# mhrice/RemFx

Hardware: AMD Instinct MI355X
Metric: audio-seconds/sec fwd+bwd (whole job) (higher is better)
Workload: dtype bf16 (fp32 accumulate); 1 GPU; Hybrid Demucs (cfg/model/demucs.yaml) train step, +exp=chorus_aug model=demucs; clips_per_gpu=64, global_batch=64, clip_samples=262144, parallelism=dp1, rccl_ranks=0, ranks=1, streams=4

## Files before the change

include/remfx_hip.h:

```cpp
#ifndef REMFX_HIP_H
#define REMFX_HIP_H

#include <stdint.h>

#ifdef __cplusplus
extern "C" {
#endif

#define RFX_ABI_VERSION 1

enum rfx_act {
  RFX_ACT_NONE = 0,
  RFX_ACT_RELU = 1,
  RFX_ACT_GELU = 2,
  RFX_ACT_TANH = 3,
  RFX_ACT_PRELU = 4,
  RFX_ACT_LEAKY = 5,
  RFX_ACT_SIGMOID = 6
};

typedef struct rfx_ktab_entry {
  int32_t off;
  int32_t da;
  int32_t db;
  int32_t flags;
} rfx_ktab_entry;

typedef struct rfx_gemm_desc {
  int32_t N, M, K;
  int32_t OA, OB;
  int32_t IA, IB;
  int32_t SA, SB;
  int32_t Mpad, Kpad;
  int32_t out_a0, out_b0, out_sa, out_sb;
  int32_t R;
  int32_t mg_log, mg_axis, mg_len, mg_off;
  int32_t Kpad_t, gpt, ntaps, gpt2;
  int64_t in_ns, in_as, in_bs;
  int64_t out_ns, out_cs, out_as, out_bs;
  int64_t in_cs, in_extent;
  int32_t in_bf16, out_bf16;
  int32_t halo_nt, halo_rows, halo_w, halo_da0, halo_db0, halo_pad;
} rfx_gemm_desc;

typedef struct rfx_epilogue {
  const float* bias;
  int32_t act;
  const float* act_param;
  const float* res;
  int64_t res_ns, res_cs, res_as, res_bs;
  int32_t act2;
  int32_t bwd;
  float* gparam;
  double* stat_sums;
  int32_t stat_slots;
  float* glu_out;
  int64_t glu_ns;
} rfx_epilogue;

enum rfx_gemm_prec { RFX_PREC_F32 = 0, RFX_PREC_BF16X3 = 1, RFX_PREC_BF16 = 2 };

int rfx_pack_a(const float* w, const int32_t* woff, int64_t w_ms, int32_t M, int32_t K,
               int32_t Mpad, int32_t Kpad, int32_t prec, float* apack, void* stream);
int rfx_unpack_add(const float* dapack, const int32_t* woff, int64_t w_ms, int32_t M, int32_t K,
                   int32_t Kpad, float* dw, int32_t splits, void* stream);
int rfx_unpack_add_bias(const float* dapack, const int32_t* woff, int64_t w_ms, int32_t M, int32_t K, int32_t Kpad, float* dw,
                        int32_t bias_col, float* db, int32_t splits, void* stream);
int rfx_unpack_set(const float* dapack, const int32_t* woff, int64_t w_ms, int32_t M, int32_t K,
                   int32_t Kpad, float* dw, int32_t splits, void* stream);
int rfx_unpack_col(const float* dapack, int32_t M, int32_t Kpad, int32_t col, int32_t splits, float* out, void* stream);

int rfx_gemm_fwd(const rfx_gemm_desc* d, const float* apack, const rfx_ktab_entry* ktab,
                 const float* in, float* out, const rfx_epilogue* epi,
                 const float* apack2, const rfx_ktab_entry* ktab2, int32_t K2, int32_t Kpad2,
                 const float* in2 ,
                 int32_t prec ,
                 void* stream);

int rfx_gemm_wgrad(const rfx_gemm_desc* d, const rfx_ktab_entry* ktab, const float* in,
                   const float* g, float* dapack, int64_t ws_floats, int32_t* splits_out, int32_t prec, void* stream);

enum rfx_stft_out {
  RFX_STFT_COMPLEX = 0,
  RFX_STFT_CAC = 1,
  RFX_STFT_MAG = 2,
  RFX_STFT_POW = 3,
  RFX_STFT_MAGPOW = 4,
  RFX_STFT_COMPLEX_FM = 5
};
typedef struct rfx_stft_desc {
  int32_t R, T;
  int32_t n_fft, hop, win;
  int32_t bins;
  int32_t frame0;
  int32_t frames_out;
  int32_t mode;
  int32_t extra_pad_l, extra_pad_r;
  int32_t in_mode;
  int32_t in_offset;
  int32_t herm;
  float scale;
  float eps, alpha;
  int32_t accum;
} rfx_stft_desc;

int rfx_fft_analysis(const rfx_stft_desc* d, const float* x, const float* window, const float* mul,
                     float* out, void* stream);
int64_t rfx_fft_synthesis_ws(const rfx_stft_desc* d);
int rfx_fft_synthesis(const rfx_stft_desc* d, const float* spec, const float* window, const float* mul,
                      float* ws, float* out, void* stream);

int rfx_lstm_pack_bytes(int32_t H);
int rfx_lstm_ws_bytes(int32_t H);
int rfx_lstm_pack(const float* whh, int32_t H, void* pack, void* stream);
int rfx_lstm_cat_params(const float* w_ih, const float* w_ih_r, const float* b_ih, const float* b_hh, const float* b_ih_r,
                        const float* b_hh_r, int32_t H, int32_t Cin, float* wcat, float* bcat, void* stream);
int rfx_lstm_grad_scatter(const float* dwcat, const float* dbcat, int32_t H, int32_t Cin, float* g_w_ih, float* g_w_ih_r,
                          float* g_b_ih, float* g_b_hh, float* g_b_ih_r, float* g_b_hh_r, void* stream);
int rfx_lstm_local(int32_t H, int32_t Bn, int32_t prec, int32_t bwd);
int rfx_lstm_pack_local(const float* whh, int32_t H, void* pack, void* stream);
int rfx_lstm_fwd(const float* xp, const void* pack, int32_t T, int32_t Bn, int32_t H, float* out, float* gates,
                 float* cstate, void* ws, int32_t prec, void* stream);
int rfx_lstm_bwd(const float* gout, const void* pack, const float* gates, const float* cstate, int32_t T,
                 int32_t Bn, int32_t H, float* dG, void* ws, int32_t prec, void* stream);
int rfx_lstm_set_local(int32_t fwd_max_sequences, int32_t bwd_max_sequences);

int rfx_act_fwd(const float* x, float* y, int64_t n, int32_t act, void* stream);
int rfx_act_bwd(const float* x, const float* gy, float* gx, int64_t n, int32_t act, void* stream);
int rfx_act_add_fwd(const float* x, const float* res, float* y, int64_t n, int32_t act, void* stream);
int rfx_act_rows(const float* x, int64_t xs0, int64_t xs1, int64_t xs2, const float* gy, int64_t gs0, int64_t gs1,
                 int64_t gs2, float* out, int64_t os0, int64_t os1, int64_t os2, int32_t D0, int32_t D1, int32_t D2,
                 int32_t T, int32_t act, void* stream);
int rfx_act_rows16(const void* x, int64_t xs0, int64_t xs1, int64_t xs2, const float* gy, int64_t gs0, int64_t gs1,
                   int64_t gs2, void* out, int64_t os0, int64_t os1, int64_t os2, int32_t D0, int32_t D1, int32_t D2,
                   int32_t T, int32_t act, void* stream);
int rfx_mul(const float* a, const float* b, float* y, int64_t n, void* stream);
int rfx_prelu_fwd(const float* x, const float* slope, float* y, int64_t N, int64_t C, int64_t L, void* stream);
int rfx_prelu_bwd(const float* x, const float* gy, const float* slope, float* gx, double* ws, float* gslope,
                  int64_t N, int64_t C, int64_t L, void* stream);

int64_t rfx_channel_sum_ws(const float* x, int32_t N, int32_t C, int32_t A, int32_t B, int64_t ns, int64_t cs, int64_t as, int64_t bs);
int rfx_channel_sum(const float* x, int32_t N, int32_t C, int32_t A, int32_t B, int64_t ns, int64_t cs,
                    int64_t as, int64_t bs, double* ws, float* out, void* stream);

int rfx_add_bcast(const float* x, const float* y, float* out, int64_t N, int32_t C, int32_t A, int32_t B,
                  int64_t yn, int64_t yc, int64_t ya, int64_t yb, float alpha, void* stream);
int rfx_row_moments_slots(int64_t L);
int rfx_row_moments(const float* x, int32_t R, int64_t L, double* sums, float* mean, float* stdv, float eps, float* coef_a,
                    float* coef_b, void* stream);
int rfx_row_affine(const float* x, const float* a, const float* b, float* out, int32_t R, int64_t L, void* stream);

int rfx_dropout(const float* x, float* out, int64_t n, float p, uint64_t seed, void* stream);

int rfx_span_mask(float* x, int32_t R, int32_t F, int32_t T, const int32_t* f0, const int32_t* f1, const int32_t* t0,
                  const int32_t* t1, void* stream);

int rfx_blstm_frames(const float* src, const float* skip, float* dst, int32_t B, int32_t C, int32_t T, int32_t nfr,
                     int32_t width, int32_t stride, int32_t mode, void* stream);

#define RFX_L1_SLOTS 512
int rfx_l1_sum(const float* a, const float* b, int64_t n, double* ws, float scale, float* out, void* stream);

int rfx_localstate_fwd(const float* q, const float* k, const float* cont, const float* qd, int32_t B, int32_t heads,
                       int32_t ch, int32_t T, int32_t nd, float* w, float* out, void* stream);
int rfx_localstate_bwd(const float* q, const float* k, const float* cont, const float* qd, const float* w,
                       const float* gout, int32_t B, int32_t heads, int32_t ch, int32_t T, int32_t nd, float* dq, float* dk,
                       float* dcont, float* dqd, void* stream);

int rfx_localstate_mfma_ok(int32_t B, int32_t heads, int32_t ch, int32_t T, int32_t nd);
int rfx_localstate_mfma_fwd(const float* q, const float* k, const float* cont, const float* qd, int32_t B, int32_t heads,
                            int32_t ch, int32_t T, int32_t nd, float* out, void* stream);
int rfx_localstate_mfma_bwd(const float* q, const float* k, const float* cont, const float* qd, const float* gout, int32_t B,
                            int32_t heads, int32_t ch, int32_t T, int32_t nd, float* dq, float* dk, float* dcont, float* dqd,
                            float* stat , void* stream);
int rfx_localstate_gen_fwd(const float* q, const float* k, const float* cont, const float* qd, int32_t B, int32_t heads,
                           int32_t ch, int32_t T, int32_t nd, float* stat, float* out, void* stream);
int rfx_localstate_gen_bwd(const float* q, const float* k, const float* cont, const float* qd, float* stat, const float* out,
                           const float* gout, int32_t B, int32_t heads, int32_t ch, int32_t T, int32_t nd, float* dq, float* dk,
                           float* dcont, float* dqd, void* stream);

int rfx_fx_distortion(const float* x, float* y, int32_t B, int64_t T, const float* gain , void* stream);
int rfx_fx_delay(const float* x, float* y, int32_t B, int64_t T, const int32_t* delay_samples, const float* feedback,
                 const float* mix, void* stream);
int rfx_fx_chorus(const float* x, float* y, int32_t B, int64_t T, float sample_rate, const float* rate_hz, const float* depth,
                  const float* centre_delay_ms, const float* feedback, const float* mix, void* stream);
int rfx_fx_compressor(const float* x, float* y, float* env_ws , int32_t B, int64_t T,
                      const float* threshold_lin, const float* ratio, const float* c_attack, const float* c_release, void* stream);
int rfx_fx_reverb(const float* x, float* y, int32_t B, int64_t T, int32_t sample_rate, const float* damp, const float* feedback,
                  const float* wet1, const float* dry, void* stream);
int rfx_fx_loudness(const float* x, int32_t B, int64_t T, int32_t chunk, int32_t hop_len, int32_t nhop, int32_t nblk,
                    double inv_block, const double* coef, float target_lufs, double* hop_ws, float* lufs, float* gain, void* stream);
int rfx_fx_scale(const float* x, float* y, int32_t B, int64_t T, const float* gain, void* stream);

int rfx_dconv_layer_ok(int32_t C, int32_t T, int32_t dil);
int rfx_dconv_layer_fwd(const float* x, float* out, int32_t N, int32_t C, int32_t T, int32_t dil, const float* w1, const float* b1,
                        const float* gn1w, const float* gn1b, const float* w2, const float* b2, const float* gn2w,
                        const float* gn2b, const float* scale, float eps, void* h16, void* z16, float* a_out, float* stats,
                        void* stream);
int rfx_dconv_layer_bwd_rows(int32_t N);
int rfx_dconv_layer_bwd(const float* x, const float* g, float* gx, int32_t N, int32_t C, int32_t T, int32_t dil, const float* w1,
                        const float* b1, const float* gn1w, const float* gn1b, const float* w2, const float* b2, const float* gn2w,
                        const float* gn2b, const float* scale, float eps, void* dz_bf16, float* a_out, void* dh_bf16, float* partial,
                        void* stream);

int rfx_gemm_fwd_variant(const rfx_gemm_desc* d, const rfx_epilogue* epi, int32_t two_phase, int32_t prec);

int rfx_mha_fwd(const float* q, const float* k, const float* v, int32_t B, int32_t heads, int32_t ch, int32_t T, float* stat,
                float* out, void* stream);
int rfx_mha_bwd(const float* q, const float* k, const float* v, float* stat, const float* out, const float* gout, int32_t B,
                int32_t heads, int32_t ch, int32_t T, float* dq, float* dk, float* dv, void* stream);

int rfx_groupnorm_fwd(const float* x, const float* gamma, const float* beta, int32_t N, int32_t C, int32_t S,
                      int32_t G, float eps, int32_t mode, const float* res, const float* scale,
                      double* sums ,
                      int32_t sums_given, float* mean, float* rstd, float* y, void* stream);
int rfx_groupnorm_stat_chunks(int32_t C, int32_t S, int32_t G);
int64_t rfx_norm_bwd_work_floats(int32_t N, int32_t C, int32_t S, int32_t G);
int rfx_groupnorm_bwd(const float* x, const float* gamma, const float* beta, const float* mean,
                      const float* rstd, const float* gy, int32_t N, int32_t C, int32_t S, int32_t G,
                      int32_t mode, const float* scale, float* work, float* dx, float* dgamma, float* dbeta,
                      float* dscale, void* stream);

int rfx_groupnorm_fwd_x16(const void* x, const float* gamma, const float* beta, int32_t N, int32_t C, int32_t S, int32_t G,
                          float eps, int32_t mode, const float* res, const float* scale, double* sums, int32_t sums_given,
                          float* mean, float* rstd, float* y, void* stream);
int rfx_groupnorm_bwd_x16(const void* x, const float* gamma, const float* beta, const float* mean, const float* rstd,
                          const float* gy, int32_t N, int32_t C, int32_t S, int32_t G, int32_t mode, const float* scale,
                          float* work, void* dx, float* dgamma, float* dbeta, float* dscale, void* stream);
int rfx_batchnorm_stat_slots(int32_t N, int32_t S);
int rfx_batchnorm_fwd(const float* x, const float* gamma, const float* beta, int32_t N, int32_t C, int32_t S,
                      float eps, int32_t mode, int32_t use_given_stats, double* sums, float* mean, float* rstd,
                      float* y, void* stream);
int rfx_batchnorm_bwd(const float* x, const float* gamma, const float* beta, const float* mean,
                      const float* rstd, const float* gy, int32_t N, int32_t C, int32_t S, int32_t mode,
                      float* work, float* dx, float* dgamma, float* dbeta, void* stream);
int rfx_avgpool2d_fwd(const float* x, float* y, int64_t NC, int32_t H, int32_t W, int32_t kh, int32_t kw,
                      void* stream);
int rfx_avgpool2d_bwd(const float* gy, float* gx, int64_t NC, int32_t H, int32_t W, int32_t kh, int32_t kw,
                      void* stream);
int rfx_glu_fwd(const float* x, float* y, int64_t N, int64_t C, int64_t S, void* stream);
int rfx_glu_bwd(const float* x, const float* gy, float* gx, int64_t N, int64_t C, int64_t S, void* stream);
int rfx_glu_bwd_bf16(const void* x, const float* gy, void* gx, int64_t N, int64_t C, int64_t S, void* stream);

int64_t rfx_cplx_slots(int32_t N, int64_t S);
int rfx_cplx_moments(const float* x, int32_t N, int32_t C, int64_t S, double* ws, double* sums, void* stream);
int rfx_cplx_coef_fwd(const double* sums, double inv_count, const float* stats_in, const float* Wrr, const float* Wri,
                      const float* Wii, const float* Br, const float* Bi, float eps, int32_t C, float* coef, float* stats_out,
                      float* RMr, float* RMi, float* RVrr, float* RVri, float* RVii, float momentum, void* stream);
int rfx_cplx_coef_bwd(const double* sums, double inv_count, const float* stats_in, const float* Wrr, const float* Wri,
                      const float* Wii, const float* Br, const float* Bi, float eps, int32_t C, const float* gcoef, float* gw,
                      float* cm, void* stream);
int rfx_cplx_moments_bwd(const float* x, const float* coef, int32_t N, int32_t C, int64_t S, float* gx, void* stream);
int rfx_cplx_affine_act_fwd(const float* x, const float* coef, int32_t N, int32_t C, int64_t S, float slope,
                            float* out, int64_t out_ns, int64_t out_im_off, void* stream);
int rfx_cplx_affine_act_bwd(const float* x, const float* coef, const float* gy, int64_t gy_ns, int64_t gy_im_off,
                            int32_t N, int32_t C, int64_t S, float slope, float* gx, double* ws, float* gcoef, void* stream);
int rfx_bound_mask_fwd(const float* m, const float* tf, float* out, int32_t N, int64_t P, int64_t m_ns,
                       int64_t tf_ns, int64_t out_ns, void* stream);
int rfx_bound_mask_bwd(const float* m, const float* tf, const float* gout, float* gm, int32_t N, int64_t P,
                       int64_t m_ns, int64_t tf_ns, int64_t g_ns, int64_t gm_ns, void* stream);

int rfx_phase_mask_fwd(const float* mag, const float* xc, float* out, int64_t n, void* stream);
int rfx_phase_mask_bwd(const float* xc, const float* gout, float* gmag, int64_t n, void* stream);

#define RFX_STFT_REDUCE_SLOTS 64
int rfx_stft_loss_reduce(const float* xc, const float* yc, int32_t R, int64_t n, float eps, double* ws, float* sums,
                         void* stream);
int rfx_stft_loss_grad(const float* xc, const float* yc, int32_t R, int64_t n, float eps,
                       const float* sums, float w_sc, float w_lm, const float* gup, float* gxc, void* stream);
int64_t rfx_stft_pair_loss_ws(const rfx_stft_desc* d);
int rfx_stft_pair_loss(const rfx_stft_desc* d, const float* x, const float* y, const float* window, float eps, double* ws, float* sums,
                       float* xspec, float* ymag, void* stream);
int rfx_stft_loss_grad_m(const float* xc, const float* ymag, int32_t R, int64_t n, float eps, const float* sums, float w_sc,
                         float w_lm, const float* gup, float* gxc, void* stream);
int rfx_fft_synthesis_lossgrad(const rfx_stft_desc* d, const float* xspec, const float* ymag, const float* sums, float w_sc,
                               float w_lm, float eps, const float* gup, const float* window, float* ws, float* out, void* stream);
int rfx_l1_grad(const float* a, const float* b, int64_t n, float w, const float* gup, float* g, void* stream);
#define RFX_SISDR_SLOTS 128
int rfx_sisdr_sums(const float* x, const float* t, int32_t R, int64_t L, int64_t x_rs, int64_t t_rs,
                   double* ws, double* sums, void* stream);
int rfx_sisdr_finish(const double* sums, int32_t R, int64_t L, int32_t zero_mean, double eps, float* out, void* stream);
int rfx_mrstft_combine(const float* const* sums, const int64_t* n, int32_t nres, int32_t R, int32_t per_example_sc, float* out,
                       void* stream);

int rfx_zero(void* p, int64_t nbytes, void* stream);
#define RFX_SUMSQ_SLOTS 4096
int rfx_sumsq(const float* g, int64_t n, double* ws, double* out, void* stream);
int rfx_clip_coef(const double* sumsq, float max_norm, float pre, float* coef, float* norm_out, void* stream);
int rfx_adamw_step(float* p, const float* g, float* m, float* v, int64_t n, float lr, float b1, float b2,
                   float eps, float wd, int32_t step, const float* gscale, void* stream);

typedef struct rfx_cl_tensor {
  void* p;
  int64_t ns, as;
  int32_t bs, c0;
} rfx_cl_tensor;

enum rfx_cl_epi {
  RFX_CL_STORE = 0,
  RFX_CL_GELU = 1,
  RFX_CL_GLU = 2,
  RFX_CL_DGELU = 3,
  RFX_CL_STORE_CM = 5,
  RFX_CL_DGLU = 4
};

typedef struct rfx_cl_conv_desc {
  rfx_cl_tensor in;
  int32_t N, IA, IB, OA, OB, SA;
  int32_t NTR, NCH, NTC, KS;
  int32_t da0, da_step;
  int32_t db0, db_step;
  int32_t wrapb;
  const void* apack;
  int32_t M, BM;
  int32_t mode;
  int32_t G, g_off, OAo, Co;
  const float* bias;
  const float* rowadd;
  rfx_cl_tensor out0, out1, aux0, res;
  void* cm_out;
  int64_t cm_ns, cm_cs, cm_as;
  int32_t cm_fold;
} rfx_cl_conv_desc;
int rfx_cl_conv(const rfx_cl_conv_desc* d, void* stream);
int rfx_cl_pack(const float* src, const int32_t* idx, int64_t n, void* dst, void* stream);
int rfx_cl_from_cm(const void* src, int32_t src_bf16, int64_t s_ns, int64_t s_cs, int64_t s_as, int32_t N, int32_t C, int32_t A,
                   int32_t B, const rfx_cl_tensor* dst, const rfx_cl_tensor* res, const rfx_cl_tensor* aux, int32_t mode, void* stream);
int rfx_cl_to_cm(const rfx_cl_tensor* src, int32_t N, int32_t C, int32_t A, int32_t B, void* dst, int32_t dst_bf16, int64_t d_ns,
                 int64_t d_cs, int64_t d_as, const void* aux16, void* stream);
int rfx_cl_im2col_s4(const float* src, int64_t s_ns, int64_t s_cs, int64_t s_as, int32_t N, int32_t Cs, int32_t IA, int32_t IB, int32_t OA,
                     int32_t OB, int32_t along_b, void* dst, void* stream);
int rfx_cl_im2col_fm(const float* src, const float* coef_a, const float* coef_b, int32_t N, int32_t F, int32_t bins, void* dst, void* stream);
int rfx_fm_cm_affine(const float* in, float* out, const float* coef_a, const float* coef_b, int32_t N, int32_t bins, int32_t F, int32_t to_fm,
                     void* stream);
int rfx_cl_dgelu(const void* g, const void* z, void* out, int64_t n, void* stream);
int rfx_cl_dglu(const void* g, const void* zab, void* out, int64_t npos, int32_t C, void* stream);

typedef struct rfx_cl_wgrad_desc {
  rfx_cl_tensor p, q;
  int32_t N, OA, IA, B;
  int32_t SA, da0, NTR;
  int32_t NTC, db0, db_step;
  int32_t M, Cq, CW;
  int32_t RW, WK;
  int32_t S, ahead, bias;
  int32_t PW;
  float* ws;
} rfx_cl_wgrad_desc;
int64_t rfx_cl_wgrad_ws_floats(const rfx_cl_wgrad_desc* d);
int rfx_cl_wgrad(const rfx_cl_wgrad_desc* d, void* stream);
int rfx_cl_wgrad_reduce(const float* ws, const int32_t* map, int64_t nmap, int32_t S, int32_t DT, int32_t RW, int32_t WK, float* dw,
                        int64_t wn, float* db, int32_t accumulate, void* stream);

typedef struct rfx_cl_dconv_desc {
  const void* x;
  const void* gy;
  void* y;
  void* a; void* hpre; float* stats;
  void* dz; void* dh; float* partial;
  const void* w1p; const void* w2p; const void* w2dp; const void* w1dp;
  const float *b1, *g1w, *g1b, *b2, *g2w, *g2b, *scale;
  int32_t S, C, H, dil, grid, x_or_gy_ok;
  float eps;
  int32_t TPS;
  float* tsum; float* sums;
  float* pg_dst[5];
} rfx_cl_dconv_desc;
int rfx_cl_dconv_ok(int32_t C, int32_t H, int32_t T, int32_t backward);
int rfx_cl_dconv_fwd(const rfx_cl_dconv_desc* d, void* stream);
int rfx_cl_dconv_bwd(const rfx_cl_dconv_desc* d, float* pgrad, void* stream);

int rfx_cl_rowsum(const rfx_cl_tensor* x, int32_t N, int32_t A, int32_t B, int32_t C, int32_t G, float scale, float* partial, float* out,
                  int32_t accumulate, void* stream);

int rfx_abi_version(void);
int rfx_gemm_pick_r(int32_t M, int32_t K);

#ifdef __cplusplus
}
#endif
#endif
```

remfx_amd/_lib.py:

```python
import ctypes as C
import glob
import os
import subprocess

_HERE = os.path.dirname(os.path.abspath(__file__))
_ROOT = os.path.dirname(_HERE)
CSRC = os.path.join(_HERE, "csrc")
INCLUDE = os.path.join(_ROOT, "include")
LIBDIR = os.path.join(_HERE, "_C")
LIBPATH = os.environ.get("RFX_LIBPATH_DEV") or os.path.join(LIBDIR, "libremfx_hip.so")

HIPCC_FLAGS = ["--offload-arch=gfx950", "-O3", "-std=c++17", "-fPIC", "-ffp-contract=fast",
               "-I" + INCLUDE, "-I" + CSRC]


def sources():
    return sorted(glob.glob(os.path.join(CSRC, "*.hip")))


def _stale():
    if not os.path.exists(LIBPATH):
        return True
    t = os.path.getmtime(LIBPATH)
    deps = sources() + glob.glob(os.path.join(CSRC, "*.h")) + glob.glob(os.path.join(INCLUDE, "*.h"))
    return any(os.path.getmtime(p) > t for p in deps)


def build(force=False, verbose=False):
    if not force and not _stale():
        return LIBPATH
    hipcc = os.environ.get("HIPCC", "/opt/rocm/bin/hipcc")
    os.makedirs(LIBDIR, exist_ok=True)
    objs = []
    hdr_t = max([os.path.getmtime(p) for p in glob.glob(os.path.join(CSRC, "*.h")) +
                 glob.glob(os.path.join(INCLUDE, "*.h"))] or [0])
    procs = []
    for src in sources():
        obj = os.path.join(LIBDIR, os.path.basename(src)[:-4] + ".o")
        objs.append(obj)
        if (not force and os.path.exists(obj) and os.path.getmtime(obj) > os.path.getmtime(src)
                and os.path.getmtime(obj) > hdr_t):
            continue
        cmd = [hipcc] + HIPCC_FLAGS + ["-c", src, "-o", obj]
        if verbose:
            print(" ".join(cmd))
        procs.append((src, subprocess.Popen(cmd, stdout=subprocess.PIPE, stderr=subprocess.STDOUT)))
    for src, p in procs:
        out, _ = p.communicate()
        if p.returncode != 0:
            raise RuntimeError(f"hipcc failed on {src}:\n{out.decode()}")
    cmd = [hipcc, "--offload-arch=gfx950", "-shared", "-fPIC", "-o", LIBPATH] + objs
    r = subprocess.run(cmd, stdout=subprocess.PIPE, stderr=subprocess.STDOUT)
    if r.returncode != 0:
        raise RuntimeError(f"link failed:\n{r.stdout.decode()}")
    return LIBPATH


class KtabEntry(C.Structure):
    _fields_ = [("off", C.c_int32), ("da", C.c_int32), ("db", C.c_int32), ("flags", C.c_int32)]


class GemmDesc(C.Structure):
    _fields_ = [(n, C.c_int32) for n in ("N", "M", "K", "OA", "OB", "IA", "IB", "SA", "SB", "Mpad",
                                         "Kpad", "out_a0", "out_b0", "out_sa", "out_sb", "R", "mg_log", "mg_axis", "mg_len", "mg_off",
                                         "Kpad_t", "gpt", "ntaps", "gpt2")] + \
               [(n, C.c_int64) for n in ("in_ns", "in_as", "in_bs", "out_ns", "out_cs", "out_as", "out_bs", "in_cs", "in_extent")] + \
               [("in_bf16", C.c_int32), ("out_bf16", C.c_int32)] + \
               [(n, C.c_int32) for n in ("halo_nt", "halo_rows", "halo_w", "halo_da0", "halo_db0", "halo_pad")]


class Epilogue(C.Structure):
    _fields_ = [("bias", C.c_void_p), ("act", C.c_int32), ("act_param", C.c_void_p),
                ("res", C.c_void_p), ("res_ns", C.c_int64), ("res_cs", C.c_int64),
                ("res_as", C.c_int64), ("res_bs", C.c_int64), ("act2", C.c_int32), ("bwd", C.c_int32),
                ("gparam", C.c_void_p), ("stat_sums", C.c_void_p), ("stat_slots", C.c_int32),
                ("glu_out", C.c_void_p), ("glu_ns", C.c_int64)]


class StftDesc(C.Structure):
    _fields_ = [(n, C.c_int32) for n in ("R", "T", "n_fft", "hop", "win", "bins", "frame0", "frames_out",
                                         "mode", "extra_pad_l", "extra_pad_r", "in_mode", "in_offset",
                                         "herm")] + \
               [(n, C.c_float) for n in ("scale", "eps", "alpha")] + [("accum", C.c_int32)]


class ClTensor(C.Structure):
    _fields_ = [("p", C.c_void_p), ("ns", C.c_int64), ("as_", C.c_int64), ("bs", C.c_int32), ("c0", C.c_int32)]


class ClConvDesc(C.Structure):
    _fields_ = [("inp", ClTensor)] + \
               [(n, C.c_int32) for n in ("N", "IA", "IB", "OA", "OB", "SA", "NTR", "NCH", "NTC", "KS", "da0", "da_step", "db0",
                                         "db_step", "wrapb")] + \
               [("apack", C.c_void_p)] + \
               [(n, C.c_int32) for n in ("M", "BM", "mode", "G", "g_off", "OAo", "Co")] + \
               [("bias", C.c_void_p), ("rowadd", C.c_void_p), ("out0", ClTensor), ("out1", ClTensor), ("aux0", ClTensor), ("res", ClTensor),
                ("cm_out", C.c_void_p), ("cm_ns", C.c_int64), ("cm_cs", C.c_int64), ("cm_as", C.c_int64), ("cm_fold", C.c_int32)]


class ClDconvDesc(C.Structure):
    _fields_ = [(n, C.c_void_p) for n in ("x", "gy", "y", "a", "hpre", "stats", "dz", "dh", "partial", "w1p", "w2p", "w2dp", "w1dp",
                                          "b1", "g1w", "g1b", "b2", "g2w", "g2b", "scale")] + \
               [(n, C.c_int32) for n in ("S", "C", "H", "dil", "grid", "x_or_gy_ok")] + [("eps", C.c_float), ("TPS", C.c_int32), ("tsum", C.c_void_p), ("sums", C.c_void_p), ("pg_dst", C.c_void_p * 5)]


class ClWgradDesc(C.Structure):
    _fields_ = [("p", ClTensor), ("q", ClTensor)] + \
               [(n, C.c_int32) for n in ("N", "OA", "IA", "B", "SA", "da0", "NTR", "NTC", "db0", "db_step", "M", "Cq", "CW", "RW", "WK",
                                         "S", "ahead", "bias", "PW")] + \
               [("ws", C.c_void_p)]


_P, _I32, _I64 = C.c_void_p, C.c_int32, C.c_int64
SIGNATURES = {
    "rfx_abi_version": [],
    "rfx_gemm_pick_r": [_I32, _I32],
    "rfx_pack_a": [_P, _P, _I64, _I32, _I32, _I32, _I32, _I32, _P, _P],
    "rfx_unpack_add": [_P, _P, _I64, _I32, _I32, _I32, _P, _I32, _P],
    "rfx_unpack_add_bias": [_P, _P, _I64, _I32, _I32, _I32, _P, _I32, _P, _I32, _P],
    "rfx_unpack_set": [_P, _P, _I64, _I32, _I32, _I32, _P, _I32, _P],
    "rfx_unpack_col": [_P, _I32, _I32, _I32, _I32, _P, _P],
    "rfx_gemm_fwd": [C.POINTER(GemmDesc), _P, _P, _P, _P, C.POINTER(Epilogue), _P, _P, _I32, _I32, _P, _I32, _P],
    "rfx_gemm_fwd_variant": [C.POINTER(GemmDesc), C.POINTER(Epilogue), _I32, _I32],
    "rfx_gemm_wgrad": [C.POINTER(GemmDesc), _P, _P, _P, _P, _I64, C.POINTER(C.c_int32), _I32, _P],
    "rfx_fft_analysis": [C.POINTER(StftDesc), _P, _P, _P, _P, _P],
    "rfx_fft_synthesis_ws": [C.POINTER(StftDesc)],
    "rfx_fft_synthesis": [C.POINTER(StftDesc), _P, _P, _P, _P, _P, _P],
    "rfx_stft_loss_reduce": [_P, _P, _I32, _I64, C.c_float, _P, _P, _P],
    "rfx_stft_loss_grad": [_P, _P, _I32, _I64, C.c_float, _P, C.c_float, C.c_float, _P, _P, _P],
    "rfx_stft_loss_grad_m": [_P, _P, _I32, _I64, C.c_float, _P, C.c_float, C.c_float, _P, _P, _P],
    "rfx_stft_pair_loss_ws": [C.POINTER(StftDesc)],
    "rfx_stft_pair_loss": [C.POINTER(StftDesc), _P, _P, _P, C.c_float, _P, _P, _P, _P, _P],
    "rfx_fft_synthesis_lossgrad": [C.POINTER(StftDesc), _P, _P, _P, C.c_float, C.c_float, C.c_float, _P, _P, _P, _P, _P],
    "rfx_l1_grad": [_P, _P, _I64, C.c_float, _P, _P, _P],
    "rfx_sisdr_sums": [_P, _P, _I32, _I64, _I64, _I64, _P, _P, _P],
    "rfx_sisdr_finish": [_P, _I32, _I64, _I32, C.c_double, _P, _P],
    "rfx_mrstft_combine": [_P, _P, _I32, _I32, _I32, _P, _P],
    "rfx_zero": [_P, _I64, _P],
    "rfx_sumsq": [_P, _I64, _P, _P, _P],
    "rfx_clip_coef": [_P, C.c_float, C.c_float, _P, _P, _P],
    "rfx_adamw_step": [_P, _P, _P, _P, _I64, C.c_float, C.c_float, C.c_float, C.c_float, C.c_float, _I32, _P, _P],
    "rfx_groupnorm_stat_chunks": [_I32, _I32, _I32],
    "rfx_norm_bwd_work_floats": [_I32, _I32, _I32, _I32],
    "rfx_batchnorm_stat_slots": [_I32, _I32],
    "rfx_groupnorm_fwd": [_P, _P, _P, _I32, _I32, _I32, _I32, C.c_float, _I32, _P, _P, _P, _I32, _P, _P, _P, _P],
    "rfx_groupnorm_bwd": [_P, _P, _P, _P, _P, _P, _I32, _I32, _I32, _I32, _I32, _P, _P, _P, _P, _P, _P, _P],
    "rfx_groupnorm_fwd_x16": [_P, _P, _P, _I32, _I32, _I32, _I32, C.c_float, _I32, _P, _P, _P, _I32, _P, _P, _P, _P],
    "rfx_groupnorm_bwd_x16": [_P, _P, _P, _P, _P, _P, _I32, _I32, _I32, _I32, _I32, _P, _P, _P, _P, _P, _P, _P],
    "rfx_batchnorm_fwd": [_P, _P, _P, _I32, _I32, _I32, C.c_float, _I32, _I32, _P, _P, _P, _P, _P],
    "rfx_batchnorm_bwd": [_P, _P, _P, _P, _P, _P, _I32, _I32, _I32, _I32, _P, _P, _P, _P, _P],
    "rfx_avgpool2d_fwd": [_P, _P, _I64, _I32, _I32, _I32, _I32, _P],
    "rfx_avgpool2d_bwd": [_P, _P, _I64, _I32, _I32, _I32, _I32, _P],
    "rfx_cplx_slots": [_I32, _I64],
    "rfx_cplx_moments": [_P, _I32, _I32, _I64, _P, _P, _P],
    "rfx_cplx_moments_bwd": [_P, _P, _I32, _I32, _I64, _P, _P],
    "rfx_cplx_coef_fwd": [_P, C.c_double, _P, _P, _P, _P, _P, _P, C.c_float, _I32, _P, _P, _P, _P, _P, _P, _P, C.c_float, _P],
    "rfx_cplx_coef_bwd": [_P, C.c_double, _P, _P, _P, _P, _P, _P, C.c_float, _I32, _P, _P, _P, _P],
    "rfx_cplx_affine_act_fwd": [_P, _P, _I32, _I32, _I64, C.c_float, _P, _I64, _I64, _P],
    "rfx_cplx_affine_act_bwd": [_P, _P, _P, _I64, _I64, _I32, _I32, _I64, C.c_float, _P, _P, _P, _P],
    "rfx_bound_mask_fwd": [_P, _P, _P, _I32, _I64, _I64, _I64, _I64, _P],
    "rfx_bound_mask_bwd": [_P, _P, _P, _P, _I32, _I64, _I64, _I64, _I64, _I64, _P],
    "rfx_phase_mask_fwd": [_P, _P, _P, _I64, _P],
    "rfx_phase_mask_bwd": [_P, _P, _P, _I64, _P],
    "rfx_glu_fwd": [_P, _P, _I64, _I64, _I64, _P],
    "rfx_glu_bwd": [_P, _P, _P, _I64, _I64, _I64, _P],
    "rfx_glu_bwd_bf16": [_P, _P, _P, _I64, _I64, _I64, _P],
    "rfx_act_fwd": [_P, _P, _I64, _I32, _P],
    "rfx_act_bwd": [_P, _P, _P, _I64, _I32, _P],
    "rfx_act_add_fwd": [_P, _P, _P, _I64, _I32, _P],
    "rfx_act_rows": [_P, _I64, _I64, _I64, _P, _I64, _I64, _I64, _P, _I64, _I64, _I64, _I32, _I32, _I32, _I32, _I32, _P],
    "rfx_act_rows16": [_P, _I64, _I64, _I64, _P, _I64, _I64, _I64, _P, _I64, _I64, _I64, _I32, _I32, _I32, _I32, _I32, _P],
    "rfx_mul": [_P, _P, _P, _I64, _P],
    "rfx_prelu_fwd": [_P, _P, _P, _I64, _I64, _I64, _P],
    "rfx_prelu_bwd": [_P, _P, _P, _P, _P, _P, _I64, _I64, _I64, _P],
    "rfx_l1_sum": [_P, _P, _I64, _P, C.c_float, _P, _P],
    "rfx_add_bcast": [_P, _P, _P, _I64, _I32, _I32, _I32, _I64, _I64, _I64, _I64, C.c_float, _P],
    "rfx_localstate_fwd": [_P, _P, _P, _P, _I32, _I32, _I32, _I32, _I32, _P, _P, _P],
    "rfx_localstate_bwd": [_P, _P, _P, _P, _P, _P, _I32, _I32, _I32, _I32, _I32, _P, _P, _P, _P, _P],
    "rfx_dconv_layer_ok": [_I32, _I32, _I32],
    "rfx_dconv_layer_bwd_rows": [_I32],
    "rfx_dconv_layer_bwd": [_P, _P, _P, _I32, _I32, _I32, _I32, _P, _P, _P, _P, _P, _P, _P, _P, _P, C.c_float, _P, _P, _P, _P, _P],
    "rfx_dconv_layer_fwd": [_P, _P, _I32, _I32, _I32, _I32, _P, _P, _P, _P, _P, _P, _P, _P, _P, C.c_float, _P, _P, _P, _P, _P],
    "rfx_fx_distortion": [_P, _P, _I32, _I64, _P, _P],
    "rfx_fx_delay": [_P, _P, _I32, _I64, _P, _P, _P, _P],
    "rfx_fx_chorus": [_P, _P, _I32, _I64, C.c_float, _P, _P, _P, _P, _P, _P],
    "rfx_fx_compressor": [_P, _P, _P, _I32, _I64, _P, _P, _P, _P, _P],
    "rfx_fx_reverb": [_P, _P, _I32, _I64, _I32, _P, _P, _P, _P, _P],
    "rfx_fx_loudness": [_P, _I32, _I64, _I32, _I32, _I32, _I32, C.c_double, _P, C.c_float, _P, _P, _P, _P],
    "rfx_fx_scale": [_P, _P, _I32, _I64, _P, _P],
    "rfx_localstate_gen_fwd": [_P, _P, _P, _P, _I32, _I32, _I32, _I32, _I32, _P, _P, _P],
    "rfx_localstate_gen_bwd": [_P, _P, _P, _P, _P, _P, _P, _I32, _I32, _I32, _I32, _I32, _P, _P, _P, _P, _P],
    "rfx_mha_fwd": [_P, _P, _P, _I32, _I32, _I32, _I32, _P, _P, _P],
    "rfx_mha_bwd": [_P, _P, _P, _P, _P, _P, _I32, _I32, _I32, _I32, _P, _P, _P, _P],
    "rfx_localstate_mfma_ok": [_I32, _I32, _I32, _I32, _I32],
    "rfx_localstate_mfma_fwd": [_P, _P, _P, _P, _I32, _I32, _I32, _I32, _I32, _P, _P],
    "rfx_localstate_mfma_bwd": [_P, _P, _P, _P, _P, _I32, _I32, _I32, _I32, _I32, _P, _P, _P, _P, _P, _P],
    "rfx_blstm_frames": [_P, _P, _P, _I32, _I32, _I32, _I32, _I32, _I32, _I32, _P],
    "rfx_span_mask": [_P, _I32, _I32, _I32, _P, _P, _P, _P, _P],
    "rfx_dropout": [_P, _P, _I64, C.c_float, C.c_uint64, _P],
    "rfx_row_moments_slots": [_I64],
    "rfx_row_moments": [_P, _I32, _I64, _P, _P, _P, C.c_float, _P, _P, _P],
    "rfx_row_affine": [_P, _P, _P, _P, _I32, _I64, _P],
    "rfx_lstm_pack_bytes": [_I32],
    "rfx_lstm_pack": [_P, _I32, _P, _P],
    "rfx_lstm_cat_params": [_P, _P, _P, _P, _P, _P, _I32, _I32, _P, _P, _P],
    "rfx_lstm_grad_scatter": [_P, _P, _I32, _I32, _P, _P, _P, _P, _P, _P, _P],
    "rfx_lstm_local": [_I32, _I32, _I32, _I32],
    "rfx_lstm_pack_local": [_P, _I32, _P, _P],
    "rfx_lstm_ws_bytes": [_I32],
    "rfx_lstm_fwd": [_P, _P, _I32, _I32, _I32, _P, _P, _P, _P, _I32, _P],
    "rfx_lstm_bwd": [_P, _P, _P, _P, _I32, _I32, _I32, _P, _P, _I32, _P],
    "rfx_lstm_set_local": [_I32, _I32],
    "rfx_channel_sum_ws": [_P, _I32, _I32, _I32, _I32, _I64, _I64, _I64, _I64],
    "rfx_channel_sum": [_P, _I32, _I32, _I32, _I32, _I64, _I64, _I64, _I64, _P, _P, _P],
    "rfx_cl_conv": [C.POINTER(ClConvDesc), _P],
    "rfx_cl_pack": [_P, _P, _I64, _P, _P],
    "rfx_cl_wgrad_ws_floats": [_P],
    "rfx_cl_wgrad": [_P, _P],
    "rfx_cl_wgrad_reduce": [_P, _P, _I64, _I32, _I32, _I32, _I32, _P, _I64, _P, _I32, _P],
    "rfx_cl_from_cm": [_P, _I32, _I64, _I64, _I64, _I32, _I32, _I32, _I32, C.POINTER(ClTensor), C.POINTER(ClTensor), C.POINTER(ClTensor),
                       _I32, _P],
    "rfx_cl_rowsum": [C.POINTER(ClTensor), _I32, _I32, _I32, _I32, _I32, C.c_float, _P, _P, _I32, _P],
    "rfx_cl_to_cm": [C.POINTER(ClTensor), _I32, _I32, _I32, _I32, _P, _I32, _I64, _I64, _I64, _P, _P],
    "rfx_cl_dgelu": [_P, _P, _P, _I64, _P],
    "rfx_cl_dglu": [_P, _P, _P, _I64, _I32, _P],
    "rfx_cl_im2col_s4": [_P, _I64, _I64, _I64, _I32, _I32, _I32, _I32, _I32, _I32, _I32, _P, _P],
    "rfx_cl_im2col_fm": [_P, _P, _P, _I32, _I32, _I32, _P, _P],
    "rfx_fm_cm_affine": [_P, _P, _P, _P, _I32, _I32, _I32, _I32, _P],
    "rfx_cl_dconv_ok": [_I32, _I32, _I32, _I32],
    "rfx_cl_dconv_fwd": [_P, _P],
    "rfx_cl_dconv_bwd": [_P, _P, _P],
}

_RET64 = {"rfx_cl_wgrad_ws_floats", "rfx_cplx_slots", "rfx_norm_bwd_work_floats", "rfx_stft_pair_loss_ws", "rfx_channel_sum_ws", "rfx_fft_synthesis_ws"}
_lib = None


def lib():
    global _lib
    if _lib is not None:
        return _lib
    import torch
    if not os.path.exists(LIBPATH):
        raise RuntimeError(
            f"{LIBPATH} not found: run `python -c 'import __graft_entry__ as g; g.build()'` "
            "(hipcc --offload-arch=gfx950).  remfx_amd has no CPU fallback.")
    L = C.CDLL(LIBPATH)
    for name, argtypes in SIGNATURES.items():
        fn = getattr(L, name)
        fn.argtypes = argtypes
        fn.restype = C.c_int64 if name in _RET64 else C.c_int
    if L.rfx_abi_version() != 1:
        raise RuntimeError("libremfx_hip ABI version mismatch")
    _lib = L
    return L


def check(rc, what):
    if rc != 0:
        raise RuntimeError(f"{what} failed with code {rc}")
```

remfx_amd/csrc/lstm.hip:

```cpp
#include "common.h"
#include <stdlib.h>

typedef __bf16 bf16x8 __attribute__((ext_vector_type(8)));

__device__ __forceinline__ uint32_t lstm_bf16_rne(float f) {
  const uint32_t u = __float_as_uint(f);
  return (u + 0x7fffu + ((u >> 16) & 1u)) >> 16;
}
__device__ __forceinline__ float lstm_sigmoid(float x) { return __builtin_amdgcn_rcpf(1.f + __expf(-x)); }
__device__ __forceinline__ float lstm_tanh(float x) { return 2.f * __builtin_amdgcn_rcpf(1.f + __expf(-2.f * x)) - 1.f; }
__device__ __forceinline__ void split_hi_lo(float v, unsigned short& hi, unsigned short& lo) {
  const uint32_t u = __float_as_uint(v);
  const float r = v - __uint_as_float(u & 0xffff0000u);
  hi = (unsigned short)(u >> 16);
  lo = (unsigned short)((__float_as_uint(r) + 0x8000u) >> 16);
}

__global__ void lstm_pack_kernel(const float* __restrict__ whh, int H, uint4* __restrict__ fwdA, uint4* __restrict__ bwdA) {
  const int nub = H / 32, nks = H / 16, nks4 = 4 * H / 16;
  const int64_t nf = (int64_t)nub * 4 * nks * 64, nb = (int64_t)nub * nks4 * 64;
  for (int64_t idx = (int64_t)blockIdx.x * blockDim.x + threadIdx.x; idx < nf + nb; idx += (int64_t)gridDim.x * blockDim.x) {
    uint32_t hi[4] = {0, 0, 0, 0}, lo[4] = {0, 0, 0, 0};
    const bool f = idx < nf;
    const int64_t i = f ? idx : idx - nf;
    const int lane = (int)(i & 63);
    int64_t r = i >> 6;
#pragma unroll
    for (int q = 0; q < 8; ++q) {
      float v;
      if (f) {
        const int ks = (int)(r % nks), tl = (int)((r / nks) % 2), ub = (int)(r / (2 * nks)), m = lane & 31;
        v = whh[(int64_t)((2 * tl + (m >> 4)) * H + 16 * ub + (m & 15)) * H + 16 * ks + 8 * (lane >> 5) + q];
      } else {
        const int ks = (int)(r % nks4), ub = (int)(r / nks4);
        v = whh[(int64_t)(16 * ks + 8 * (lane >> 5) + q) * H + 32 * ub + (lane & 31)];
      }
      const uint32_t h = lstm_bf16_rne(v);
      const uint32_t l = lstm_bf16_rne(v - __uint_as_float(h << 16));
      hi[q >> 1] |= h << (16 * (q & 1));
      lo[q >> 1] |= l << (16 * (q & 1));
    }
    uint4* dst = f ? fwdA : bwdA;
    const int64_t n = f ? nf : nb;
    dst[i] = make_uint4(hi[0], hi[1], hi[2], hi[3]);
    dst[n + i] = make_uint4(lo[0], lo[1], lo[2], lo[3]);
  }
}


#define RFX_LSTM_MAX_WAVES 768
#define RFX_LSTM_SPIN_LIMIT (1 << 22)

struct LstmArgs {
  const float* xp;
  const uint4* packA;
  float* out;
  float* gates;
  float* cstate;
  const float* gout;
  float* dG;
  uint64_t* xch;
  uint32_t* ctr;
  int32_t* err;
  int64_t pack_stride;
  int T, Bn, H, P;
  int tile0, nclusters;
};

__device__ __forceinline__ bool lstm_wait(const uint32_t* ctr, uint32_t target) {
  for (int it = 0; it < RFX_LSTM_SPIN_LIMIT; ++it) {
    const uint32_t v = __hip_atomic_load(ctr, __ATOMIC_RELAXED, __HIP_MEMORY_SCOPE_AGENT);
    if (__builtin_amdgcn_readfirstlane(v) >= target) return true;
    __builtin_amdgcn_s_sleep(1);
  }
  return false;
}
__device__ __forceinline__ void lstm_arrive(uint32_t* ctr, int lane) {
  __builtin_amdgcn_s_waitcnt(0x0F70);
  if (lane == 0) __hip_atomic_fetch_add(ctr, 1u, __ATOMIC_RELAXED, __HIP_MEMORY_SCOPE_AGENT);
}
__device__ __forceinline__ bf16x8 lstm_xch_load(const uint64_t* p) {
  const uint64_t a = __hip_atomic_load(p, __ATOMIC_RELAXED, __HIP_MEMORY_SCOPE_AGENT);
  const uint64_t b = __hip_atomic_load(p + 1, __ATOMIC_RELAXED, __HIP_MEMORY_SCOPE_AGENT);
  const uint4 v = make_uint4((uint32_t)a, (uint32_t)(a >> 32), (uint32_t)b, (uint32_t)(b >> 32));
  return __builtin_bit_cast(bf16x8, v);
}
__device__ __forceinline__ void lstm_xch_store(uint64_t* phi, uint64_t* plo, float v0, float v1, float v2, float v3) {
  unsigned short h0, h1, h2, h3, l0, l1, l2, l3;
  split_hi_lo(v0, h0, l0); split_hi_lo(v1, h1, l1); split_hi_lo(v2, h2, l2); split_hi_lo(v3, h3, l3);
  const uint64_t hi = (uint64_t)h0 | ((uint64_t)h1 << 16) | ((uint64_t)h2 << 32) | ((uint64_t)h3 << 48);
  const uint64_t lo = (uint64_t)l0 | ((uint64_t)l1 << 16) | ((uint64_t)l2 << 32) | ((uint64_t)l3 << 48);
  __hip_atomic_store(phi, hi, __ATOMIC_RELAXED, __HIP_MEMORY_SCOPE_AGENT);
  __hip_atomic_store(plo, lo, __ATOMIC_RELAXED, __HIP_MEMORY_SCOPE_AGENT);
}

__device__ __forceinline__ bool lstm_ids(const LstmArgs& a, int nwc, int& cluster, int& ub) {
  const int w = blockIdx.x, j = w >> 3;
  cluster = (j / nwc) * 8 + (w & 7);
  ub = j % nwc;
  return cluster < a.nclusters;
}

typedef uint32_t lstm_u32x4 __attribute__((ext_vector_type(4)));
typedef const __attribute__((address_space(1))) lstm_u32x4* lstm_gptr_t;

struct LstmAFrag { uint4 h[2], l[2]; };

extern __shared__ __attribute__((aligned(16))) unsigned char lstm_smem[];

__device__ __forceinline__ void lstm_fetch_lds(const uint64_t* src, int n, int lane) {
  for (int i = 0; i < n; ++i)
    __builtin_amdgcn_global_load_lds((const __attribute__((address_space(1))) void*)(src + (i * 64 + lane) * 2),
                                     (__attribute__((address_space(3))) void*)(lstm_smem + i * 1024), 16, 0,
                                     16 );
}

__device__ __forceinline__ void lstm_fetch_lds_hi(const uint64_t* src, int nks, int lane) {
  for (int ks = 0; ks < nks; ++ks)
    __builtin_amdgcn_global_load_lds((const __attribute__((address_space(1))) void*)(src + (2 * ks * 64 + lane) * 2),
                                     (__attribute__((address_space(3))) void*)(lstm_smem + ks * 2048), 16, 0,
                                     16 );
}
__device__ __forceinline__ void lstm_xch_store_hi(uint64_t* phi, float v0, float v1, float v2, float v3) {
  const uint64_t hi = (uint64_t)rfx_cvt_pk_bf16(v0, v1) | ((uint64_t)rfx_cvt_pk_bf16(v2, v3) << 32);
  __hip_atomic_store(phi, hi, __ATOMIC_RELAXED, __HIP_MEMORY_SCOPE_AGENT);
}

template <int D, int NKS, bool LO>
__global__ __launch_bounds__(64) __attribute__((amdgpu_waves_per_eu(1, 1))) void lstm_fwd_kernel(const LstmArgs a) {
  int cluster, ub;
  if (!lstm_ids(a, a.H / 16, cluster, ub)) return;
  const int H = a.H, Bn = a.Bn, T = a.T, P = a.P;
  const int dir = cluster & 1, row0 = (a.tile0 + (cluster >> 1)) * 32;
  const int lane = threadIdx.x, l31 = lane & 31, hh = lane >> 5;
  const int nks = NKS ? NKS : H / 16, nwc = nks;
  const int row = row0 + l31;
  const bool rvalid = row < Bn;
  const int rowc = rvalid ? row : 0;
  const float* __restrict__ xp = a.xp + (int64_t)dir * 4 * H * P;
  const int nf = nwc * 2 * nks * 64;
  uint64_t abase = (uint64_t)(a.packA + (int64_t)dir * a.pack_stride + ub * 2 * nks * 64);
  lstm_gptr_t Ahi = (lstm_gptr_t)abase;
  lstm_gptr_t Alo = Ahi + nf;
  float* outp = a.out + (int64_t)dir * H * P;
  float* gsave = a.gates ? a.gates + (int64_t)dir * 4 * H * P : nullptr;
  float* csave = a.gates ? a.cstate + (int64_t)dir * H * P : nullptr;
  const int bufw = nks * 256;
  uint64_t* xch = a.xch + (int64_t)cluster * 2 * bufw;
  uint32_t* ctr = a.ctr + cluster * 16;
  const uint32_t uP = (uint32_t)P, HP = (uint32_t)H * uP;
  const uint32_t ubase = (uint32_t)(16 * ub + 4 * hh) * uP + (uint32_t)rowc;
  const uint32_t lane16 = (uint32_t)lane * 16u;
  auto loadA = [&](LstmAFrag& f, int ks) {
#pragma unroll
    for (int tl = 0; tl < 2; ++tl) {
      f.h[tl] = __builtin_bit_cast(uint4, *(lstm_gptr_t)((uint64_t)(Ahi + (tl * nks + ks) * 64) + lane16));
      if (LO) f.l[tl] = __builtin_bit_cast(uint4, *(lstm_gptr_t)((uint64_t)(Alo + (tl * nks + ks) * 64) + lane16));
    }
  };
  auto loadB = [&](bf16x8& bh, bf16x8& bl, int ks) {
    bh = *reinterpret_cast<const bf16x8*>(lstm_smem + ks * 2048 + lane * 16);
    if (LO) bl = *reinterpret_cast<const bf16x8*>(lstm_smem + ks * 2048 + 1024 + lane * 16);
  };
  auto mma = [&](f32x16* acc, const LstmAFrag& f, const bf16x8 bh, const bf16x8 bl) {
#pragma unroll
    for (int tl = 0; tl < 2; ++tl)
      acc[tl] = __builtin_amdgcn_mfma_f32_32x32x16_bf16(__builtin_bit_cast(bf16x8, f.h[tl]), bh, acc[tl], 0, 0, 0);
    if (LO) {
#pragma unroll
      for (int tl = 0; tl < 2; ++tl)
        acc[tl] = __builtin_amdgcn_mfma_f32_32x32x16_bf16(__builtin_bit_cast(bf16x8, f.h[tl]), bl, acc[tl], 0, 0, 0);
#pragma unroll
      for (int tl = 0; tl < 2; ++tl)
        acc[tl] = __builtin_amdgcn_mfma_f32_32x32x16_bf16(__builtin_bit_cast(bf16x8, f.l[tl]), bh, acc[tl], 0, 0, 0);
    }
  };
  float c[8];
#pragma unroll
  for (int r = 0; r < 8; ++r) c[r] = 0.f;
  f32x16 acc[2];
  LstmAFrag f[D];
#pragma unroll
  for (int d = 0; d < D; ++d) loadA(f[d], d);
  float xpv[4][8];
  {
    const uint32_t o0 = ubase + (uint32_t)((dir == 0 ? 0 : T - 1) * Bn);
#pragma unroll
    for (int g = 0; g < 4; ++g)
#pragma unroll
      for (int r = 0; r < 8; ++r) xpv[g][r] = xp[o0 + (uint32_t)g * HP + (uint32_t)((r & 3) + 8 * (r >> 2)) * uP];
  }
  for (int s = 0; s < T; ++s) {
    if (NKS) { asm volatile("" : "+s"(abase)); Ahi = (lstm_gptr_t)abase; Alo = Ahi + nf; }

    const int t = dir == 0 ? s : T - 1 - s;
    const uint32_t o0 = ubase + (uint32_t)(t * Bn);
#pragma unroll
    for (int tl = 0; tl < 2; ++tl)
#pragma unroll
      for (int r = 0; r < 16; ++r) acc[tl][r] = 0.f;
    if (s > 0) {
      if (!lstm_wait(ctr, (uint32_t)(nwc * s))) { *a.err = 1; return; }
      if (LO) lstm_fetch_lds(xch + ((s - 1) & 1) * bufw, 2 * nks, lane);
      else lstm_fetch_lds_hi(xch + ((s - 1) & 1) * bufw, nks, lane);
      __builtin_amdgcn_s_waitcnt(0x0F70);
    }
    if (s > 0) {
      bf16x8 bh[2], bl[2];
      loadB(bh[0], bl[0], 0);
      auto kstep = [&](int ks) {
#pragma unroll
        for (int d = 0; d < D; ++d) {
          const int k1 = ks + d + 1 == nks ? 0 : ks + d + 1;
          loadB(bh[(d + 1) & 1], bl[(d + 1) & 1], k1);
          mma(acc, f[d], bh[d & 1], bl[d & 1]);
          if (!(NKS && D == NKS)) {
            const int kn = ks + d + D;
            loadA(f[d], kn >= nks ? kn - nks : kn);
          }
          __builtin_amdgcn_sched_barrier(0);
        }
      };
      if (NKS) {
#pragma unroll
        for (int ks = 0; ks < NKS; ks += D) kstep(ks);
      } else {
        for (int ks = 0; ks < nks; ks += D) kstep(ks);
      }
    }
    uint64_t* hw = xch + (s & 1) * bufw;
    float hv[8], gi[8], gf[8], gc[8], go[8];
#pragma unroll
    for (int r = 0; r < 8; ++r) {
      const float ig = lstm_sigmoid(acc[0][r] + xpv[0][r]), fg = lstm_sigmoid(acc[0][r + 8] + xpv[1][r]);
      const float gg = lstm_tanh(acc[1][r] + xpv[2][r]), og = lstm_sigmoid(acc[1][r + 8] + xpv[3][r]);
      c[r] = fg * c[r] + ig * gg;
      hv[r] = og * lstm_tanh(c[r]);
      gi[r] = ig; gf[r] = fg; gc[r] = gg; go[r] = og;
    }
    if (s + 1 < T) {
#pragma unroll
      for (int hb2 = 0; hb2 < 2; ++hb2) {
        const int r0 = 4 * hb2;
        uint64_t* d = hw + ((ub * 2) * 64 + l31 + 32 * hb2) * 2 + hh;
        if (LO) lstm_xch_store(d, d + 128, hv[r0], hv[r0 + 1], hv[r0 + 2], hv[r0 + 3]);
        else lstm_xch_store_hi(d, hv[r0], hv[r0 + 1], hv[r0 + 2], hv[r0 + 3]);
      }
      lstm_arrive(ctr, lane);
    }
    if (rvalid) {
#pragma unroll
      for (int r = 0; r < 8; ++r) {
        const uint32_t o = o0 + (uint32_t)((r & 3) + 8 * (r >> 2)) * uP;
        outp[o] = hv[r];
        if (gsave) {
          gsave[o] = gi[r]; gsave[o + HP] = gf[r]; gsave[o + 2 * HP] = gc[r]; gsave[o + 3 * HP] = go[r];
          csave[o] = c[r];
        }
      }
    }
    if (s + 1 < T) {
      const uint32_t on = ubase + (uint32_t)((dir == 0 ? s + 1 : T - 2 - s) * Bn);
#pragma unroll
      for (int g = 0; g < 4; ++g)
#pragma unroll
        for (int r = 0; r < 8; ++r) xpv[g][r] = xp[on + (uint32_t)g * HP + (uint32_t)((r & 3) + 8 * (r >> 2)) * uP];
    }
  }
}

template <int TPC, int NWC, bool LO, bool RES>
__global__ __launch_bounds__(64) __attribute__((amdgpu_waves_per_eu(1, 1))) void lstm_bwd_kernel(const LstmArgs a) {
  static_assert(!RES || NWC > 0, "resident weights need the compile-time tile count");
  int cluster, ub;
  if (!lstm_ids(a, a.H / 16, cluster, ub)) return;
  const int H = a.H, Bn = a.Bn, T = a.T, P = a.P;
  const int dir = cluster & 1, row0 = (a.tile0 + (cluster >> 1)) * 32;
  const int lane = threadIdx.x, l31 = lane & 31, hh = lane >> 5;
  const int nwc = NWC ? NWC : H / 32, nwv = 2 * nwc, nks = nwv, nks4 = 4 * nks;
  const int row = row0 + l31;
  const bool rvalid = row < Bn;
  const int rowc = rvalid ? row : 0;
  const int nf = nwc * 4 * nks * 64, nb = nwc * nks4 * 64;
  uint64_t abase = (uint64_t)(a.packA + (int64_t)dir * a.pack_stride + 2 * nf + ub * 64);
  lstm_gptr_t Ahi = (lstm_gptr_t)abase;
  lstm_gptr_t Alo = Ahi + nb;
  const float* __restrict__ gates = a.gates + (int64_t)dir * 4 * H * P;
  const float* __restrict__ cst = a.cstate + (int64_t)dir * H * P;
  float* __restrict__ dG = a.dG + (int64_t)dir * 4 * H * P;
  const float* __restrict__ goutp = a.gout + (int64_t)dir * H * P;
  const int bufw = nwv * nwv * 256;
  uint64_t* xch = a.xch + (int64_t)cluster * 2 * bufw;
  uint32_t* ctr = a.ctr + cluster * 16;
  const uint32_t uP = (uint32_t)P, HP = (uint32_t)H * uP;
  const uint32_t ubase = (uint32_t)(16 * ub + 4 * hh) * uP + (uint32_t)rowc;
  constexpr int RING = RES ? 4 * NWC : 4 * TPC;
  const int F = 4 * nwc;
  auto frag_index = [&](int fi) { const int ot = fi >> 2, g = fi & 3; return (ot * nks4 + g * nks) * 64 + lane; };
  uint4 wh[RING], wl[LO ? RING : 1];
#pragma unroll
  for (int i = 0; i < RING; ++i) {
    wh[i] = __builtin_bit_cast(uint4, Ahi[frag_index(i)]);
    if (LO) wl[i] = __builtin_bit_cast(uint4, Alo[frag_index(i)]);
  }
  float dcc[8], ct[8];
  float sg[4][8], cp[8], gy[8];
  {
    const uint32_t o0 = ubase + (uint32_t)((dir == 0 ? T - 1 : 0) * Bn);
    const uint32_t op0 = ubase + (uint32_t)((T > 1 ? (dir == 0 ? T - 2 : 1) : (dir == 0 ? T - 1 : 0)) * Bn);
#pragma unroll
    for (int r = 0; r < 8; ++r) {
      const uint32_t du = (uint32_t)((r & 3) + 8 * (r >> 2)) * uP;
      dcc[r] = 0.f;
      ct[r] = cst[o0 + du];
      sg[0][r] = gates[o0 + du]; sg[1][r] = gates[o0 + du + HP]; sg[2][r] = gates[o0 + du + 2 * HP]; sg[3][r] = gates[o0 + du + 3 * HP];
      cp[r] = cst[op0 + du];
      gy[r] = goutp[o0 + du];
    }
  }
  for (int s = T - 1; s >= 0; --s) {
    if (NWC && !RES) { asm volatile("" : "+s"(abase)); Ahi = (lstm_gptr_t)abase; Alo = Ahi + nb; }
    const int step = T - 1 - s;
    const int t = dir == 0 ? s : T - 1 - s;
    const uint32_t o0 = ubase + (uint32_t)(t * Bn);
    if (step > 0) {
      if (!lstm_wait(ctr, (uint32_t)(nwv * step))) { *a.err = 1; return; }
      lstm_fetch_lds(xch + ((step - 1) & 1) * bufw + ub * nwv * 256, 2 * nwv, lane);
      __builtin_amdgcn_s_waitcnt(0x0F70);
    }
    if (step > 0) {
      for (int p = 0; p < nwv; ++p)
#pragma unroll
        for (int jj = 0; jj < 2; ++jj) {
          const f32x4 v = *reinterpret_cast<const f32x4*>(lstm_smem + (p * 2 + jj) * 1024 + lane * 16);
          gy[4 * jj] += v[0]; gy[4 * jj + 1] += v[1]; gy[4 * jj + 2] += v[2]; gy[4 * jj + 3] += v[3];
        }
    }
#pragma unroll
    for (int r = 0; r < 8; ++r) {
      const float ig = sg[0][r], fg = sg[1][r], gg = sg[2][r], og = sg[3][r];
      const float cprev = s > 0 ? cp[r] : 0.f;
      const float th = lstm_tanh(ct[r]);
      const float dc = gy[r] * og * (1.f - th * th) + dcc[r];
      sg[3][r] = gy[r] * th * og * (1.f - og);
      sg[0][r] = dc * gg * ig * (1.f - ig);
      sg[1][r] = dc * cprev * fg * (1.f - fg);
      sg[2][r] = dc * ig * (1.f - gg * gg);
      dcc[r] = dc * fg;
      ct[r] = cp[r];
    }
    if (s > 0) {
      uint4 bh[4], bl[LO ? 4 : 1];
#pragma unroll
      for (int g = 0; g < 4; ++g) {
        uint32_t x0h[2], x0l[2], x1h[2], x1l[2];
#pragma unroll
        for (int e = 0; e < 2; ++e) {
          if (LO) {
            unsigned short h0, l0, h1, l1;
            split_hi_lo(sg[g][2 * e], h0, l0); split_hi_lo(sg[g][2 * e + 1], h1, l1);
            x0h[e] = (uint32_t)h0 | ((uint32_t)h1 << 16); x0l[e] = (uint32_t)l0 | ((uint32_t)l1 << 16);
            split_hi_lo(sg[g][4 + 2 * e], h0, l0); split_hi_lo(sg[g][4 + 2 * e + 1], h1, l1);
            x1h[e] = (uint32_t)h0 | ((uint32_t)h1 << 16); x1l[e] = (uint32_t)l0 | ((uint32_t)l1 << 16);
          } else {
            x0h[e] = rfx_cvt_pk_bf16(sg[g][2 * e], sg[g][2 * e + 1]);
            x1h[e] = rfx_cvt_pk_bf16(sg[g][4 + 2 * e], sg[g][4 + 2 * e + 1]);
            x0l[e] = x1l[e] = 0;
          }
        }
        uint32_t rh[2], rl[2] = {0, 0};
#pragma unroll
        for (int e = 0; e < 2; ++e) {
          rh[e] = (uint32_t)__shfl_xor((int)(hh ? x0h[e] : x1h[e]), 32, 64);
          if (LO) rl[e] = (uint32_t)__shfl_xor((int)(hh ? x0l[e] : x1l[e]), 32, 64);
        }
        bh[g] = hh ? make_uint4(rh[0], rh[1], x1h[0], x1h[1]) : make_uint4(x0h[0], x0h[1], rh[0], rh[1]);
        if (LO) bl[g] = hh ? make_uint4(rl[0], rl[1], x1l[0], x1l[1]) : make_uint4(x0l[0], x0l[1], rl[0], rl[1]);
      }
      uint64_t* gw = xch + (step & 1) * bufw;
      auto round = [&](int f0) {
        f32x16 acc[TPC];
#pragma unroll
        for (int tp = 0; tp < TPC; ++tp)
#pragma unroll
          for (int r = 0; r < 16; ++r) acc[tp][r] = 0.f;
#pragma unroll
        for (int g = 0; g < 4; ++g) {
          const bf16x8 Bh = __builtin_bit_cast(bf16x8, bh[g]), Bl = __builtin_bit_cast(bf16x8, bl[LO ? g : 0]);
#pragma unroll
          for (int tp = 0; tp < TPC; ++tp)
            acc[tp] = __builtin_amdgcn_mfma_f32_32x32x16_bf16(__builtin_bit_cast(bf16x8, wh[(RES ? f0 : 0) + tp * 4 + g]), Bh, acc[tp], 0, 0, 0);
          if (LO) {
#pragma unroll
            for (int tp = 0; tp < TPC; ++tp)
              acc[tp] = __builtin_amdgcn_mfma_f32_32x32x16_bf16(__builtin_bit_cast(bf16x8, wh[(RES ? f0 : 0) + tp * 4 + g]), Bl, acc[tp], 0, 0, 0);
#pragma unroll
            for (int tp = 0; tp < TPC; ++tp)
              acc[tp] = __builtin_amdgcn_mfma_f32_32x32x16_bf16(__builtin_bit_cast(bf16x8, wl[LO ? (RES ? f0 : 0) + tp * 4 + g : 0]), Bh, acc[tp], 0, 0, 0);
          }
          if (!RES) {
#pragma unroll
            for (int tp = 0; tp < TPC; ++tp) {
              const int i = tp * 4 + g;
              int fn = f0 + i + RING;
              fn = fn >= F ? fn - F : fn;
              wh[i] = __builtin_bit_cast(uint4, Ahi[frag_index(fn)]);
              if (LO) wl[LO ? i : 0] = __builtin_bit_cast(uint4, Alo[frag_index(fn)]);
            }
            __builtin_amdgcn_sched_barrier(0);
          }
        }
#pragma unroll
        for (int tp = 0; tp < TPC; ++tp) {
          const int ot = (f0 >> 2) + tp;
#pragma unroll
          for (int j = 0; j < 4; ++j) {
            uint64_t* d = gw + (int64_t)(((2 * ot + (j >> 1)) * nwv + ub) * 2 + (j & 1)) * 128 + lane * 2;
            const uint64_t v0 = (uint64_t)__float_as_uint(acc[tp][4 * j]) | ((uint64_t)__float_as_uint(acc[tp][4 * j + 1]) << 32);
            const uint64_t v1 = (uint64_t)__float_as_uint(acc[tp][4 * j + 2]) | ((uint64_t)__float_as_uint(acc[tp][4 * j + 3]) << 32);
            __hip_atomic_store(d, v0, __ATOMIC_RELAXED, __HIP_MEMORY_SCOPE_AGENT);
            __hip_atomic_store(d + 1, v1, __ATOMIC_RELAXED, __HIP_MEMORY_SCOPE_AGENT);
          }
        }
      };
      if (NWC) {
#pragma unroll
        for (int f0 = 0; f0 < 4 * NWC; f0 += 4 * TPC) round(f0);
      } else {
        for (int f0 = 0; f0 < F; f0 += 4 * TPC) round(f0);
      }
      lstm_arrive(ctr, lane);
    }
    if (rvalid) {
#pragma unroll
      for (int r = 0; r < 8; ++r) {
        const uint32_t o = o0 + (uint32_t)((r & 3) + 8 * (r >> 2)) * uP;
        dG[o] = sg[0][r]; dG[o + HP] = sg[1][r]; dG[o + 2 * HP] = sg[2][r]; dG[o + 3 * HP] = sg[3][r];
      }
    }
    if (s > 0) {
      const int s1 = s - 1, s2 = s1 > 0 ? s1 - 1 : 0;
      const uint32_t on = ubase + (uint32_t)((dir == 0 ? s1 : T - 1 - s1) * Bn);
      const uint32_t opn = ubase + (uint32_t)((dir == 0 ? s2 : T - 1 - s2) * Bn);
#pragma unroll
      for (int r = 0; r < 8; ++r) {
        const uint32_t du = (uint32_t)((r & 3) + 8 * (r >> 2)) * uP;
        sg[0][r] = gates[on + du]; sg[1][r] = gates[on + du + HP]; sg[2][r] = gates[on + du + 2 * HP]; sg[3][r] = gates[on + du + 3 * HP];
        cp[r] = cst[opn + du];
        gy[r] = goutp[on + du];
      }
    }
  }
}

typedef float lstm_f32x4 __attribute__((ext_vector_type(4)));

__global__ void lstm_pack_local_kernel(const float* __restrict__ whh, int H, uint4* __restrict__ dst) {
  const int nw = H / 16, nk = H / 32, nk4 = 4 * nk;
  const int64_t nf = (int64_t)nw * 4 * nk * 64, nb = (int64_t)nw * nk4 * 64;
  for (int64_t idx = (int64_t)blockIdx.x * blockDim.x + threadIdx.x; idx < nf + nb; idx += (int64_t)gridDim.x * blockDim.x) {
    const bool f = idx < nf;
    const int64_t i = f ? idx : idx - nf;
    const int lane = (int)(i & 63), row = lane & 15, kb = lane >> 4;
    int64_t r = i >> 6;
    uint32_t pk[4] = {0, 0, 0, 0};
#pragma unroll
    for (int j = 0; j < 8; ++j) {
      float v;
      if (f) {
        const int ks = (int)(r % nk), g = (int)((r / nk) % 4), w = (int)(r / (4 * nk));
        v = whh[(int64_t)(g * H + 16 * w + row) * H + 32 * ks + 8 * kb + j];
      } else {
        const int ks = (int)(r % nk4), w = (int)(r / nk4);
        v = whh[(int64_t)(32 * ks + 8 * kb + j) * H + 16 * w + row];
      }
      pk[j >> 1] |= lstm_bf16_rne(v) << (16 * (j & 1));
    }
    dst[idx] = make_uint4(pk[0], pk[1], pk[2], pk[3]);
  }
}
static int64_t lstm_local_uint4_per_dir(int H) { return (H <= 192) ? (int64_t)2 * (H / 16) * 4 * (H / 32) * 64 : 0; }

__device__ __forceinline__ void lstm_local_publish(unsigned char* buf, int k0, int sq, float v0, float v1, float v2, float v3) {
  const int ks = k0 >> 5, kk = k0 & 31;
  *reinterpret_cast<uint2*>(buf + ks * 1024 + (16 * (kk >> 3) + sq) * 16 + 2 * (kk & 7)) =
      make_uint2(rfx_cvt_pk_bf16(v0, v1), rfx_cvt_pk_bf16(v2, v3));
}
__device__ __forceinline__ void lstm_lds_barrier() { asm volatile("s_waitcnt lgkmcnt(0)\n\ts_barrier" ::: "memory"); }

template <int NW>
__global__ __launch_bounds__(64 * NW) __attribute__((amdgpu_waves_per_eu(3, 3))) void lstm_fwd_local_kernel(const LstmArgs a, const uint4* __restrict__ lpack,
                                                                                                             int64_t lstride) {
  constexpr int H = 16 * NW, NK = H / 32;
  const int cluster = blockIdx.x, dir = cluster & 1, tile = cluster >> 1;
  const int tid = threadIdx.x, w = __builtin_amdgcn_readfirstlane(tid >> 6), lane = tid & 63, sq = lane & 15, qb = lane >> 4;
  const int Bn = a.Bn, T = a.T, P = a.P;
  const int b = tile * 16 + sq;
  const bool rvalid = b < Bn;
  const int bc = rvalid ? b : 0;
  const float* __restrict__ xp = a.xp + (int64_t)dir * 4 * H * P;
  float* outp = a.out + (int64_t)dir * H * P;
  float* gsave = a.gates ? a.gates + (int64_t)dir * 4 * H * P : nullptr;
  float* csave = a.gates ? a.cstate + (int64_t)dir * H * P : nullptr;
  const uint32_t uP = (uint32_t)P, HP = (uint32_t)H * uP;
  const int u0 = 16 * w + 4 * qb;
  const uint32_t ubase = (uint32_t)u0 * uP + (uint32_t)bc;
  uint4 wf[4][NK];
  {
    const uint4* A = lpack + (int64_t)dir * lstride + (int64_t)w * 4 * NK * 64 + lane;
#pragma unroll
    for (int g = 0; g < 4; ++g)
#pragma unroll
      for (int ks = 0; ks < NK; ++ks) wf[g][ks] = A[(g * NK + ks) * 64];
  }
  float c[4] = {0.f, 0.f, 0.f, 0.f};
  float xpv[4][4];
  {
    const uint32_t o0 = ubase + (uint32_t)((dir == 0 ? 0 : T - 1) * Bn);
#pragma unroll
    for (int g = 0; g < 4; ++g)
#pragma unroll
      for (int r = 0; r < 4; ++r) xpv[g][r] = xp[o0 + (uint32_t)g * HP + (uint32_t)r * uP];
  }
  for (int s = 0; s < T; ++s) {
    const int t = dir == 0 ? s : T - 1 - s;
    const uint32_t o0 = ubase + (uint32_t)(t * Bn);
    lstm_f32x4 acc[4];
#pragma unroll
    for (int g = 0; g < 4; ++g) acc[g] = lstm_f32x4{0.f, 0.f, 0.f, 0.f};
    if (s > 0) {
      const unsigned char* hb = lstm_smem + ((s - 1) & 1) * (NK * 1024) + lane * 16;
#pragma unroll
      for (int ks = 0; ks < NK; ++ks) {
        const bf16x8 bh = *reinterpret_cast<const bf16x8*>(hb + ks * 1024);
#pragma unroll
        for (int g = 0; g < 4; ++g)
          acc[g] = __builtin_amdgcn_mfma_f32_16x16x32_bf16(__builtin_bit_cast(bf16x8, wf[g][ks]), bh, acc[g], 0, 0, 0);
      }
    }
    float hv[4], gi[4], gf[4], gc[4], go[4];
#pragma unroll
    for (int r = 0; r < 4; ++r) {
      const float ig = lstm_sigmoid(acc[0][r] + xpv[0][r]), fg = lstm_sigmoid(acc[1][r] + xpv[1][r]);
      const float gg = lstm_tanh(acc[2][r] + xpv[2][r]), og = lstm_sigmoid(acc[3][r] + xpv[3][r]);
      c[r] = fg * c[r] + ig * gg;
      hv[r] = og * lstm_tanh(c[r]);
      gi[r] = ig; gf[r] = fg; gc[r] = gg; go[r] = og;
    }
    if (s + 1 < T) {
      lstm_local_publish(lstm_smem + (s & 1) * (NK * 1024), u0, sq, hv[0], hv[1], hv[2], hv[3]);
      const uint32_t on = ubase + (uint32_t)((dir == 0 ? s + 1 : T - 2 - s) * Bn);
#pragma unroll
      for (int g = 0; g < 4; ++g)
#pragma unroll
        for (int r = 0; r < 4; ++r) xpv[g][r] = xp[on + (uint32_t)g * HP + (uint32_t)r * uP];
      lstm_lds_barrier();
    }
    if (rvalid) {
#pragma unroll
      for (int r = 0; r < 4; ++r) {
        const uint32_t o = o0 + (uint32_t)r * uP;
        outp[o] = hv[r];
        if (gsave) {
          gsave[o] = gi[r]; gsave[o + HP] = gf[r]; gsave[o + 2 * HP] = gc[r]; gsave[o + 3 * HP] = go[r];
          csave[o] = c[r];
        }
      }
    }
  }
}

template <int NW>
__global__ __launch_bounds__(64 * NW) __attribute__((amdgpu_waves_per_eu(3, 3))) void lstm_bwd_local_kernel(const LstmArgs a, const uint4* __restrict__ lpack,
                                                                                                             int64_t lstride) {
  constexpr int H = 16 * NW, NK = H / 32, NK4 = 4 * NK;
  const int cluster = blockIdx.x, dir = cluster & 1, tile = cluster >> 1;
  const int tid = threadIdx.x, w = __builtin_amdgcn_readfirstlane(tid >> 6), lane = tid & 63, sq = lane & 15, qb = lane >> 4;
  const int Bn = a.Bn, T = a.T, P = a.P;
  const int b = tile * 16 + sq;
  const bool rvalid = b < Bn;
  const int bc = rvalid ? b : 0;
  const float* __restrict__ gates = a.gates + (int64_t)dir * 4 * H * P;
  const float* __restrict__ cst = a.cstate + (int64_t)dir * H * P;
  float* __restrict__ dG = a.dG + (int64_t)dir * 4 * H * P;
  const float* __restrict__ goutp = a.gout + (int64_t)dir * H * P;
  const uint32_t uP = (uint32_t)P, HP = (uint32_t)H * uP;
  const int u0 = 16 * w + 4 * qb;
  const uint32_t ubase = (uint32_t)u0 * uP + (uint32_t)bc;
  uint4 wb[NK4];
  {
    const uint4* A = lpack + (int64_t)dir * lstride + (int64_t)NW * 4 * NK * 64 + (int64_t)w * NK4 * 64 + lane;
#pragma unroll
    for (int ks = 0; ks < NK4; ++ks) wb[ks] = A[ks * 64];
  }
  float dcc[4] = {0.f, 0.f, 0.f, 0.f}, ct[4], sg[4][4], cp[4], gy[4];
  {
    const uint32_t o0 = ubase + (uint32_t)((dir == 0 ? T - 1 : 0) * Bn);
    const uint32_t op0 = ubase + (uint32_t)((T > 1 ? (dir == 0 ? T - 2 : 1) : (dir == 0 ? T - 1 : 0)) * Bn);
#pragma unroll
    for (int r = 0; r < 4; ++r) {
      const uint32_t du = (uint32_t)r * uP;
      ct[r] = cst[o0 + du];
      sg[0][r] = gates[o0 + du]; sg[1][r] = gates[o0 + du + HP]; sg[2][r] = gates[o0 + du + 2 * HP]; sg[3][r] = gates[o0 + du + 3 * HP];
      cp[r] = cst[op0 + du];
      gy[r] = goutp[o0 + du];
    }
  }
  lstm_f32x4 rec = lstm_f32x4{0.f, 0.f, 0.f, 0.f};
  for (int s = T - 1; s >= 0; --s) {
    const int step = T - 1 - s;
    const int t = dir == 0 ? s : T - 1 - s;
    const uint32_t o0 = ubase + (uint32_t)(t * Bn);
#pragma unroll
    for (int r = 0; r < 4; ++r) {
      const float dh = gy[r] + rec[r];
      const float ig = sg[0][r], fg = sg[1][r], gg = sg[2][r], og = sg[3][r];
      const float cprev = s > 0 ? cp[r] : 0.f;
      const float th = lstm_tanh(ct[r]);
      const float dc = dh * og * (1.f - th * th) + dcc[r];
      sg[3][r] = dh * th * og * (1.f - og);
      sg[0][r] = dc * gg * ig * (1.f - ig);
      sg[1][r] = dc * cprev * fg * (1.f - fg);
      sg[2][r] = dc * ig * (1.f - gg * gg);
      dcc[r] = dc * fg;
      ct[r] = cp[r];
    }
    unsigned char* gb = lstm_smem + (step & 1) * (NK4 * 1024);
    if (s > 0) {
#pragma unroll
      for (int g = 0; g < 4; ++g) lstm_local_publish(gb, g * H + u0, sq, sg[g][0], sg[g][1], sg[g][2], sg[g][3]);
    }
    if (rvalid) {
#pragma unroll
      for (int r = 0; r < 4; ++r) {
        const uint32_t o = o0 + (uint32_t)r * uP;
        dG[o] = sg[0][r]; dG[o + HP] = sg[1][r]; dG[o + 2 * HP] = sg[2][r]; dG[o + 3 * HP] = sg[3][r];
      }
    }
    if (s > 0) {
      lstm_lds_barrier();
      lstm_f32x4 p[4];
#pragma unroll
      for (int q = 0; q < 4; ++q) p[q] = lstm_f32x4{0.f, 0.f, 0.f, 0.f};
#pragma unroll
      for (int ks = 0; ks < NK4; ++ks) {
        const bf16x8 bh = *reinterpret_cast<const bf16x8*>(gb + ks * 1024 + lane * 16);
        p[ks & 3] = __builtin_amdgcn_mfma_f32_16x16x32_bf16(__builtin_bit_cast(bf16x8, wb[ks]), bh, p[ks & 3], 0, 0, 0);
      }
      const int s1 = s - 1, s2 = s1 > 0 ? s1 - 1 : 0;
      const uint32_t on = ubase + (uint32_t)((dir == 0 ? s1 : T - 1 - s1) * Bn);
      const uint32_t opn = ubase + (uint32_t)((dir == 0 ? s2 : T - 1 - s2) * Bn);
#pragma unroll
      for (int r = 0; r < 4; ++r) {
        const uint32_t du = (uint32_t)r * uP;
        sg[0][r] = gates[on + du]; sg[1][r] = gates[on + du + HP]; sg[2][r] = gates[on + du + 2 * HP]; sg[3][r] = gates[on + du + 3 * HP];
        cp[r] = cst[opn + du];
        gy[r] = goutp[on + du];
      }
      rec = (p[0] + p[1]) + (p[2] + p[3]);
    }
  }
}

static int64_t lstm_cluster_uint4_per_dir(int H) {
  const int64_t nf = (int64_t)(H / 32) * 4 * (H / 16) * 64, nb = (int64_t)(H / 32) * (4 * H / 16) * 64;
  return 2 * nf + 2 * nb;
}
static int64_t lstm_pack_uint4_per_dir(int H) { return lstm_cluster_uint4_per_dir(H) + lstm_local_uint4_per_dir(H); }
static int lstm_local_m[2] = {-1, -1};
static int lstm_local_max_bn(bool bwd) {
  int* m = lstm_local_m;
  if (m[0] < 0) {
    const char* e = getenv("RFX_LSTM_LOCAL");
    const char* eb = getenv("RFX_LSTM_LOCAL_BWD");
    m[0] = e ? atoi(e) : 64;
    m[1] = m[0] > 0 ? (eb ? atoi(eb) : 16) : 0;
  }
  return m[bwd];
}
extern "C" int rfx_lstm_set_local(int32_t fwd_max_sequences, int32_t bwd_max_sequences) {
  if (fwd_max_sequences < 0 || bwd_max_sequences < 0) { lstm_local_m[0] = lstm_local_m[1] = -1; return 0; }
  lstm_local_m[0] = fwd_max_sequences;
  lstm_local_m[1] = fwd_max_sequences > 0 ? bwd_max_sequences : 0;
  return 0;
}
static bool lstm_local_ok(int H, int prec, int Bn, bool bwd) { return prec == RFX_PREC_BF16 && H == 192 && Bn <= lstm_local_max_bn(bwd); }
template <int NW>
static int lstm_local_launch(bool bwd, LstmArgs a, hipStream_t s) {
  constexpr int H = 16 * NW;
  const int ntiles = (a.Bn + 15) / 16;
  const uint4* lpack = a.packA + lstm_cluster_uint4_per_dir(H);
  const int64_t lstride = a.pack_stride;
  const size_t smem = (size_t)2 * (bwd ? 4 : 1) * (H / 32) * 1024;
  static bool attr[2] = {false, false};
  if (!attr[bwd]) {
    const void* k = bwd ? reinterpret_cast<const void*>(&lstm_bwd_local_kernel<NW>) : reinterpret_cast<const void*>(&lstm_fwd_local_kernel<NW>);
    if (hipFuncSetAttribute(k, hipFuncAttributeMaxDynamicSharedMemorySize, (int)smem) != hipSuccess) return -3;
    attr[bwd] = true;
  }
  if (bwd) hipLaunchKernelGGL((lstm_bwd_local_kernel<NW>), dim3(2 * ntiles), dim3(64 * NW), smem, s, a, lpack, lstride);
  else hipLaunchKernelGGL((lstm_fwd_local_kernel<NW>), dim3(2 * ntiles), dim3(64 * NW), smem, s, a, lpack, lstride);
  RFX_CHECK_LAUNCH();
  return 0;
}

static bool lstm_bad_h(int H) { return H <= 0 || H % 32 || H > 512; }
static size_t lstm_smem_bytes(int H) { return (size_t)(H / 32) * 4096; }
static int64_t lstm_ws_ctr_off() { return 256; }
static int64_t lstm_ws_xch_off(int H) { return 256 + (int64_t)(RFX_LSTM_MAX_WAVES / (H / 32)) * 64; }

extern "C" int rfx_lstm_pack_bytes(int32_t H) {
  if (lstm_bad_h(H)) return -1;
  return (int)(lstm_pack_uint4_per_dir(H) * 16);
}

extern "C" int rfx_lstm_ws_bytes(int32_t H) {
  if (lstm_bad_h(H)) return -1;
  const int64_t nwc = H / 32;
  return (int)(lstm_ws_xch_off(H) + (RFX_LSTM_MAX_WAVES / nwc) * 2 * nwc * nwc * 4096);
}

__global__ __launch_bounds__(256) void lstm_cat_kernel(const float* __restrict__ w0, const float* __restrict__ w1, const float* __restrict__ bi0,
                                                       const float* __restrict__ bh0, const float* __restrict__ bi1, const float* __restrict__ bh1,
                                                       int64_t nw, int nb, float* __restrict__ wcat, float* __restrict__ bcat) {
  const int64_t stride = (int64_t)gridDim.x * 256;
  for (int64_t i = (int64_t)blockIdx.x * 256 + threadIdx.x; i < 2 * nw; i += stride) wcat[i] = i < nw ? w0[i] : w1[i - nw];
  for (int64_t i = (int64_t)blockIdx.x * 256 + threadIdx.x; i < 2 * nb; i += stride)
    bcat[i] = i < nb ? bi0[i] + bh0[i] : bi1[i - nb] + bh1[i - nb];
}
__global__ __launch_bounds__(256) void lstm_scatter_kernel(const float* __restrict__ dwcat, const float* __restrict__ dbcat, int64_t nw, int nb,
                                                           float* __restrict__ gw0, float* __restrict__ gw1, float* __restrict__ gbi0,
                                                           float* __restrict__ gbh0, float* __restrict__ gbi1, float* __restrict__ gbh1) {
  const int64_t stride = (int64_t)gridDim.x * 256;
  for (int64_t i = (int64_t)blockIdx.x * 256 + threadIdx.x; i < 2 * nw; i += stride) {
    if (i < nw) gw0[i] += dwcat[i]; else gw1[i - nw] += dwcat[i];
  }
  for (int64_t i = (int64_t)blockIdx.x * 256 + threadIdx.x; i < 2 * nb; i += stride) {
    const float v = dbcat[i];
    if (i < nb) { gbi0[i] += v; gbh0[i] += v; } else { gbi1[i - nb] += v; gbh1[i - nb] += v; }
  }
}
extern "C" int rfx_lstm_cat_params(const float* w_ih, const float* w_ih_r, const float* b_ih, const float* b_hh, const float* b_ih_r,
                                   const float* b_hh_r, int32_t H, int32_t Cin, float* wcat, float* bcat, void* stream) {
  if (!w_ih || !w_ih_r || !b_ih || !b_hh || !b_ih_r || !b_hh_r || !wcat || !bcat || H <= 0 || Cin <= 0) return -1;
  const int64_t nw = (int64_t)4 * H * Cin;
  const int grid = (int)((2 * nw + 255) / 256 < 1024 ? (2 * nw + 255) / 256 : 1024);
  hipLaunchKernelGGL(lstm_cat_kernel, dim3(grid), dim3(256), 0, (hipStream_t)stream, w_ih, w_ih_r, b_ih, b_hh, b_ih_r, b_hh_r, nw, 4 * H, wcat, bcat);
  RFX_CHECK_LAUNCH();
  return 0;
}
extern "C" int rfx_lstm_grad_scatter(const float* dwcat, const float* dbcat, int32_t H, int32_t Cin, float* g_w_ih, float* g_w_ih_r,
                                     float* g_b_ih, float* g_b_hh, float* g_b_ih_r, float* g_b_hh_r, void* stream) {
  if (!dwcat || !dbcat || !g_w_ih || !g_w_ih_r || !g_b_ih || !g_b_hh || !g_b_ih_r || !g_b_hh_r || H <= 0 || Cin <= 0) return -1;
  const int64_t nw = (int64_t)4 * H * Cin;
  const int grid = (int)((2 * nw + 255) / 256 < 1024 ? (2 * nw + 255) / 256 : 1024);
  hipLaunchKernelGGL(lstm_scatter_kernel, dim3(grid), dim3(256), 0, (hipStream_t)stream, dwcat, dbcat, nw, 4 * H, g_w_ih, g_w_ih_r, g_b_ih, g_b_hh,
                     g_b_ih_r, g_b_hh_r);
  RFX_CHECK_LAUNCH();
  return 0;
}

extern "C" int rfx_lstm_pack(const float* whh, int32_t H, void* pack, void* stream) {
  if (!whh || !pack || lstm_bad_h(H)) return -1;
  const int64_t nf = (int64_t)(H / 32) * 4 * (H / 16) * 64;
  uint4* p = reinterpret_cast<uint4*>(pack);
  const int64_t total = lstm_cluster_uint4_per_dir(H) / 2;
  const int grid = (int)((total + 255) / 256 < 2048 ? (total + 255) / 256 : 2048);
  hipLaunchKernelGGL(lstm_pack_kernel, dim3(grid), dim3(256), 0, (hipStream_t)stream, whh, H, p, p + 2 * nf);
  RFX_CHECK_LAUNCH();
  return 0;
}

extern "C" int rfx_lstm_local(int32_t H, int32_t Bn, int32_t prec, int32_t bwd) {
  if (lstm_bad_h(H) || Bn <= 0) return 0;
  return lstm_local_ok(H, prec, Bn, bwd != 0) ? 1 : 0;
}

extern "C" int rfx_lstm_pack_local(const float* whh, int32_t H, void* pack, void* stream) {
  if (!whh || !pack || lstm_bad_h(H)) return -1;
  const int64_t nl = lstm_local_uint4_per_dir(H);
  if (nl == 0) return 0;
  uint4* p = reinterpret_cast<uint4*>(pack);
  const int gl = (int)((nl + 255) / 256 < 2048 ? (nl + 255) / 256 : 2048);
  hipLaunchKernelGGL(lstm_pack_local_kernel, dim3(gl), dim3(256), 0, (hipStream_t)stream, whh, H, p + lstm_cluster_uint4_per_dir(H));
  RFX_CHECK_LAUNCH();
  return 0;
}

template <typename K>
static int lstm_launch(K kernel, LstmArgs a, int wpc, void* ws, void* stream) {
  const int H = a.H, ntiles = (a.Bn + 31) / 32;
  int mc = 0;
  {
    static thread_local const void* seen[24];
    static thread_local int seen_mc[24], seen_h[24];
    static thread_local int nseen = 0;
    int i = 0;
    for (; i < nseen; ++i) if (seen[i] == reinterpret_cast<const void*>(kernel) && seen_h[i] == H) break;
    if (i == nseen) {
      if (nseen == 24) nseen = 0;
      int dev = 0, ncu = 0, occ = 0;
      if (hipGetDevice(&dev) != hipSuccess || hipDeviceGetAttribute(&ncu, hipDeviceAttributeMultiprocessorCount, dev) != hipSuccess ||
          hipOccupancyMaxActiveBlocksPerMultiprocessor(&occ, kernel, 64, lstm_smem_bytes(H)) != hipSuccess) return -3;
      int waves = ncu * occ;
      if (waves > RFX_LSTM_MAX_WAVES) waves = RFX_LSTM_MAX_WAVES;
      i = nseen++;
      seen[i] = reinterpret_cast<const void*>(kernel);
      seen_h[i] = H;
      seen_mc[i] = (waves / wpc) & ~7;
    }
    mc = seen_mc[i];
  }
  const int mc_ws = RFX_LSTM_MAX_WAVES / (H / 32);
  if (mc > mc_ws) mc = mc_ws & ~7;
  if (mc < 8) return -4;
  const size_t smem = lstm_smem_bytes(H);
  unsigned char* w = reinterpret_cast<unsigned char*>(ws);
  a.err = reinterpret_cast<int32_t*>(w);
  a.ctr = reinterpret_cast<uint32_t*>(w + lstm_ws_ctr_off());
  a.xch = reinterpret_cast<uint64_t*>(w + lstm_ws_xch_off(H));
  hipStream_t s = (hipStream_t)stream;
  for (int t0 = 0; t0 < ntiles; t0 += mc / 2) {
    const int nt = ntiles - t0 < mc / 2 ? ntiles - t0 : mc / 2;
    a.tile0 = t0;
    a.nclusters = 2 * nt;
    if (hipMemsetAsync(a.ctr, 0, (size_t)mc * 64, s) != hipSuccess) return -3;
    const int blocks = ((a.nclusters + 7) / 8) * 8 * wpc;
    hipLaunchKernelGGL(kernel, dim3(blocks), dim3(64), smem, s, a);
    RFX_CHECK_LAUNCH();
  }
  return 0;
}

extern "C" int rfx_lstm_fwd(const float* xp, const void* pack, int32_t T, int32_t Bn, int32_t H, float* out,
                            float* gates, float* cstate, void* ws, int32_t prec, void* stream) {
  if (!xp || !pack || !out || !ws || T <= 0 || Bn <= 0 || lstm_bad_h(H)) return -1;
  if ((gates == nullptr) != (cstate == nullptr)) return -1;
  if ((int64_t)4 * H * T * Bn >= ((int64_t)1 << 31)) return -1;
  LstmArgs a{};
  a.xp = xp; a.packA = reinterpret_cast<const uint4*>(pack); a.out = out; a.gates = gates; a.cstate = cstate;
  a.pack_stride = lstm_pack_uint4_per_dir(H); a.T = T; a.Bn = Bn; a.H = H; a.P = T * Bn;
  const int wf = H / 16;
  if (lstm_local_ok(H, prec, Bn, false)) return lstm_local_launch<12>(false, a, (hipStream_t)stream);
  if (prec == RFX_PREC_BF16) {
    if (H == 192) return lstm_launch(lstm_fwd_kernel<12, 12, false>, a, wf, ws, stream);
    if (H == 256) return lstm_launch(lstm_fwd_kernel<16, 16, false>, a, wf, ws, stream);
    if (H == 384) return lstm_launch(lstm_fwd_kernel<24, 24, false>, a, wf, ws, stream);
    return H % 64 == 0 ? lstm_launch(lstm_fwd_kernel<4, 0, false>, a, wf, ws, stream)
                       : lstm_launch(lstm_fwd_kernel<2, 0, false>, a, wf, ws, stream);
  }
  if (H == 192) return lstm_launch(lstm_fwd_kernel<12, 12, true>, a, wf, ws, stream);
  if (H == 256) return lstm_launch(lstm_fwd_kernel<4, 16, true>, a, wf, ws, stream);
  if (H == 384) return lstm_launch(lstm_fwd_kernel<4, 24, true>, a, wf, ws, stream);
  return H % 64 == 0 ? lstm_launch(lstm_fwd_kernel<4, 0, true>, a, wf, ws, stream) : lstm_launch(lstm_fwd_kernel<2, 0, true>, a, wf, ws, stream);
}

extern "C" int rfx_lstm_bwd(const float* gout, const void* pack, const float* gates, const float* cstate, int32_t T,
                            int32_t Bn, int32_t H, float* dG, void* ws, int32_t prec, void* stream) {
  if (!gout || !pack || !gates || !cstate || !dG || !ws || T <= 0 || Bn <= 0 || lstm_bad_h(H)) return -1;
  if ((int64_t)4 * H * T * Bn >= ((int64_t)1 << 31)) return -1;
  LstmArgs a{};
  a.gout = gout; a.packA = reinterpret_cast<const uint4*>(pack); a.gates = const_cast<float*>(gates);
  a.cstate = const_cast<float*>(cstate); a.dG = dG;
  a.pack_stride = lstm_pack_uint4_per_dir(H); a.T = T; a.Bn = Bn; a.H = H; a.P = T * Bn;
  const int wb = H / 16;
  if (lstm_local_ok(H, prec, Bn, true)) return lstm_local_launch<12>(true, a, (hipStream_t)stream);
  if (prec == RFX_PREC_BF16) {
    if (H == 192) return lstm_launch(lstm_bwd_kernel<3, 6, false, true>, a, wb, ws, stream);
    if (H == 256) return lstm_launch(lstm_bwd_kernel<4, 8, false, true>, a, wb, ws, stream);
    if (H == 384) return lstm_launch(lstm_bwd_kernel<4, 12, false, true>, a, wb, ws, stream);
    return (H / 32) % 2 == 0 ? lstm_launch(lstm_bwd_kernel<2, 0, false, false>, a, wb, ws, stream)
                             : lstm_launch(lstm_bwd_kernel<1, 0, false, false>, a, wb, ws, stream);
  }
  if (H == 192) return lstm_launch(lstm_bwd_kernel<3, 6, true, true>, a, wb, ws, stream);
  return (H / 32) % 2 == 0 ? lstm_launch(lstm_bwd_kernel<2, 0, true, false>, a, wb, ws, stream)
                           : lstm_launch(lstm_bwd_kernel<1, 0, true, false>, a, wb, ws, stream);
}
```

remfx_amd/lstm.py:

```python
import ctypes as C

import torch
import torch.nn.functional as F

from . import _lib, convplan, ops
from ._lib import check
from .ops import _ptr, _stream


def _pack_whh(w_hh, w_hh_r, Bn, train):
    H = w_hh.shape[1]
    L = _lib.lib()
    nb = L.rfx_lstm_pack_bytes(H)
    if nb <= 0:
        raise ValueError(f"LSTM hidden size {H} unsupported (multiple of 32, <= 512)")
    pack = torch.empty(2 * nb, device=w_hh.device, dtype=torch.uint8)
    fwd_l, bwd_l = L.rfx_lstm_local(H, Bn, ops.GEMM_PREC, 0), (train and L.rfx_lstm_local(H, Bn, ops.GEMM_PREC, 1))
    for d, w in enumerate((w_hh, w_hh_r)):
        wc = w.contiguous()
        dst = C.c_void_p(pack.data_ptr() + d * nb)
        if not (fwd_l and (bwd_l or not train)):
            check(L.rfx_lstm_pack(_ptr(wc), H, dst, _stream()), "rfx_lstm_pack")
        if fwd_l or bwd_l:
            check(L.rfx_lstm_pack_local(_ptr(wc), H, dst, _stream()), "rfx_lstm_pack_local")
    return pack


_WS = {}


def _workspace(device, H):
    key = (device.index, H, ops.raw_stream())
    ws = _WS.get(key)
    if ws is None:
        nb = _lib.lib().rfx_lstm_ws_bytes(H)
        if nb <= 0:
            raise ValueError(f"LSTM hidden size {H} unsupported (multiple of 32, <= 512)")
        ws = torch.zeros(nb, device=device, dtype=torch.uint8)
        _WS[key] = ws
    return ws


def error_flag():
    return any(bool(ws[:4].view(torch.int32).item()) for ws in _WS.values())


def _whh_plan(out4, g4, H, d, Bn):
    xs = out4[:, d * H:(d + 1) * H]
    gs = g4[:, d * 4 * H:(d + 1) * 4 * H]
    shift = -Bn if d == 0 else Bn
    key = ops._key("lstm_whh", xs.shape, xs.stride(), gs.stride(), shift)
    dp = ops._plans(key, out4.device, lambda: convplan.shift_plan(
        tuple(xs.shape), xs.stride(), 4 * H, shift, tuple(gs.shape), gs.stride()))
    return dp, xs, gs


class _LSTMLayerFn(torch.autograd.Function):

    @staticmethod
    def forward(ctx, x, w_ih, w_hh, b_ih, b_hh, w_ih_r, w_hh_r, b_ih_r, b_hh_r, T, Bn):
        ops._req(x, "x")
        H, Cin = w_hh.shape[1], w_ih.shape[1]
        P = T * Bn
        if x.shape != (1, Cin, P):
            raise ValueError(f"lstm: expected (1, {Cin}, {P}) channel-major input, got {tuple(x.shape)}")
        x = x.contiguous()
        x4 = x.unsqueeze(2)
        if x.is_cuda and all(t.is_contiguous() and t.dtype == torch.float32 for t in (w_ih, w_ih_r, b_ih, b_hh, b_ih_r, b_hh_r)):
            wcat = torch.empty((8 * H, Cin, 1, 1), device=x.device, dtype=torch.float32)
            bcat = torch.empty((8 * H,), device=x.device, dtype=torch.float32)
            check(_lib.lib().rfx_lstm_cat_params(_ptr(w_ih), _ptr(w_ih_r), _ptr(b_ih), _ptr(b_hh), _ptr(b_ih_r), _ptr(b_hh_r), H, Cin,
                                                 _ptr(wcat), _ptr(bcat), _stream()), "rfx_lstm_cat_params")
        else:
            wcat = torch.cat([w_ih, w_ih_r]).view(8 * H, Cin, 1, 1)
            bcat = torch.cat([b_ih + b_hh, b_ih_r + b_hh_r])
        xp = ops.conv2d_forward(x4, wcat, bcat, (1, 1), (0, 0), (1, 1))
        need = any(ctx.needs_input_grad)
        pack = _pack_whh(w_hh, w_hh_r, Bn, need)
        out = torch.empty((1, 2 * H, P), device=x.device, dtype=torch.float32)
        gates = torch.empty((2, 4 * H, P), device=x.device, dtype=torch.float32) if need else None
        cst = torch.empty((2, H, P), device=x.device, dtype=torch.float32) if need else None
        check(_lib.lib().rfx_lstm_fwd(_ptr(xp), _ptr(pack), T, Bn, H, _ptr(out), _ptr(gates), _ptr(cst),
                                      _ptr(_workspace(x.device, H)), ops.GEMM_PREC, _stream()),
              "rfx_lstm_fwd")
        ctx.prec = ops.GEMM_PREC
        if need:
            ctx.save_for_backward(x, wcat, pack, gates, cst, out)
            ctx.dims = (T, Bn, H, Cin)
            ctx.params = (w_ih, w_hh, b_ih, b_hh, w_ih_r, w_hh_r, b_ih_r, b_hh_r)
        return out

    @staticmethod
    def backward(ctx, g):
        x, wcat, pack, gates, cst, out = ctx.saved_tensors
        T, Bn, H, Cin = ctx.dims
        P = T * Bn
        g = g.contiguous()
        dG = torch.empty((1, 8 * H, 1, P), device=g.device, dtype=torch.float32)
        check(_lib.lib().rfx_lstm_bwd(_ptr(g), _ptr(pack), _ptr(gates), _ptr(cst), T, Bn, H, _ptr(dG),
                                      _ptr(_workspace(g.device, H)), ctx.prec, _stream()),
              "rfx_lstm_bwd")
        x4 = x.unsqueeze(2)
        dx = None
        if ctx.needs_input_grad[0]:
            dx = ops.conv2d_dgrad(dG, wcat, tuple(x4.shape), x4.stride(), (1, 1), (0, 0), (1, 1)).squeeze(2)
        sink = ops.SINK
        tg = [sink.lookup(p) for p in ctx.params] if sink is not None else [None]
        sunk = all(t is not None for t in tg)
        stream = sink.stream_for_wgrad(x, dG, out) if sunk else torch.cuda.current_stream()
        with torch.cuda.stream(stream):
            dwcat, dbcat = ops.conv2d_wgrad(x4, dG, tuple(wcat.shape), (1, 1), (0, 0), (1, 1), True)
            dwcat = dwcat.view(8 * H, Cin)
            out4 = out.unsqueeze(2)
            dwhh = []
            for d in range(2):
                dp, xs, gs = _whh_plan(out4, dG, H, d, Bn)
                dap = ops.gemm_wgrad(dp, xs, gs)
                if sunk:
                    ops.unpack_add(dp, dap, tg[1 + 4 * d][1])
                    dwhh.append(None)
                    continue
                dw = ops.zeros((4 * H, H), g.device)
                ops.unpack_add(dp, dap, dw)
                dwhh.append(dw)
            db0, db1 = dbcat[:4 * H], dbcat[4 * H:]
            grads = (dwcat[:4 * H], dwhh[0], db0, db0, dwcat[4 * H:], dwhh[1], db1, db1)
            if sunk:
                v = [t[1] for t in tg]
                check(_lib.lib().rfx_lstm_grad_scatter(_ptr(dwcat), _ptr(dbcat), H, Cin, _ptr(v[0]), _ptr(v[4]), _ptr(v[2]), _ptr(v[3]),
                                                       _ptr(v[6]), _ptr(v[7]), _stream()), "rfx_lstm_grad_scatter")
        if sunk:
            for i, _ in tg:
                sink.wrote(i)
            return (dx,) + (None,) * 10
        return (dx,) + grads + (None, None)


def blstm(module, x, T, Bn):
    if not module.bidirectional:
        raise NotImplementedError("only bidirectional LSTMs are on the hot path (cfg/model/umx.yaml, HDemucs BLSTM)")
    if not module.bias or getattr(module, "proj_size", 0):
        raise NotImplementedError("lstm: bias=True, proj_size=0 only")
    h = x
    for layer in range(module.num_layers):
        p = [getattr(module, f"{n}_l{layer}{sfx}") for sfx in ("", "_reverse")
             for n in ("weight_ih", "weight_hh", "bias_ih", "bias_hh")]
        h = _LSTMLayerFn.apply(h, *p, T, Bn)
        if module.dropout > 0 and module.training and layer < module.num_layers - 1:
            from . import nnops
            h = nnops.dropout(h, module.dropout, True)
    return h
```

Baseline: 3677 audio-seconds/sec.

## Pack LSTM saved gates and cell state into one vectorized per-unit-quad layout

Merges the separate gates and cell-state buffers into one 'saved' buffer laid out as f32x4 quads per (time, unit-group, sequence), so forward writes and backward reads use 16-byte vector accesses. The local kernels also transpose xp/out/gout/dG tiles through LDS so global accesses become contiguous rows of four sequences, with a vectorized template variant when Bn is a multiple of 4 and pointers are aligned. The default for the local LSTM path changes from enabled to disabled unless an environment variable is set, so the default run may use the cluster kernels, which only get the saved-layout change. This adds LDS traffic and wave barriers for the transposes.

```diff
diff --git a/include/remfx_hip.h b/include/remfx_hip.h
--- a/include/remfx_hip.h
+++ b/include/remfx_hip.h
@@ -119,9 +119,9 @@
                           float* g_b_ih, float* g_b_hh, float* g_b_ih_r, float* g_b_hh_r, void* stream);
 int rfx_lstm_local(int32_t H, int32_t Bn, int32_t prec, int32_t bwd);
 int rfx_lstm_pack_local(const float* whh, int32_t H, void* pack, void* stream);
-int rfx_lstm_fwd(const float* xp, const void* pack, int32_t T, int32_t Bn, int32_t H, float* out, float* gates,
-                 float* cstate, void* ws, int32_t prec, void* stream);
-int rfx_lstm_bwd(const float* gout, const void* pack, const float* gates, const float* cstate, int32_t T,
+int rfx_lstm_fwd(const float* xp, const void* pack, int32_t T, int32_t Bn, int32_t H, float* out, float* saved,
+                 void* ws, int32_t prec, void* stream);
+int rfx_lstm_bwd(const float* gout, const void* pack, const float* saved, int32_t T,
                  int32_t Bn, int32_t H, float* dG, void* ws, int32_t prec, void* stream);
 int rfx_lstm_set_local(int32_t fwd_max_sequences, int32_t bwd_max_sequences);
 
diff --git a/remfx_amd/_lib.py b/remfx_amd/_lib.py
--- a/remfx_amd/_lib.py
+++ b/remfx_amd/_lib.py
@@ -208,8 +208,8 @@
     "rfx_lstm_local": [_I32, _I32, _I32, _I32],
     "rfx_lstm_pack_local": [_P, _I32, _P, _P],
     "rfx_lstm_ws_bytes": [_I32],
-    "rfx_lstm_fwd": [_P, _P, _I32, _I32, _I32, _P, _P, _P, _P, _I32, _P],
-    "rfx_lstm_bwd": [_P, _P, _P, _P, _I32, _I32, _I32, _P, _P, _I32, _P],
+    "rfx_lstm_fwd": [_P, _P, _I32, _I32, _I32, _P, _P, _P, _I32, _P],
+    "rfx_lstm_bwd": [_P, _P, _P, _I32, _I32, _I32, _P, _P, _I32, _P],
     "rfx_lstm_set_local": [_I32, _I32],
     "rfx_channel_sum_ws": [_P, _I32, _I32, _I32, _I32, _I64, _I64, _I64, _I64],
     "rfx_channel_sum": [_P, _I32, _I32, _I32, _I32, _I64, _I64, _I64, _I64, _P, _P, _P],
diff --git a/remfx_amd/csrc/lstm.hip b/remfx_amd/csrc/lstm.hip
--- a/remfx_amd/csrc/lstm.hip
+++ b/remfx_amd/csrc/lstm.hip
@@ -55,8 +55,7 @@
   const float* xp;
   const uint4* packA;
   float* out;
-  float* gates;
-  float* cstate;
+  float* saved;
   const float* gout;
   float* dG;
   uint64_t* xch;
@@ -66,6 +65,10 @@
   int T, Bn, H, P;
   int tile0, nclusters;
 };
+
+__device__ __forceinline__ uint32_t lstm_sv_idx(int t, int g4, int H, int Bn, int b) {
+  return ((uint32_t)(t * (H / 4) + g4) * 5u) * (uint32_t)Bn + (uint32_t)b;
+}
 
 __device__ __forceinline__ bool lstm_wait(const uint32_t* ctr, uint32_t target) {
   for (int it = 0; it < RFX_LSTM_SPIN_LIMIT; ++it) {
@@ -143,8 +146,7 @@
   lstm_gptr_t Ahi = (lstm_gptr_t)abase;
   lstm_gptr_t Alo = Ahi + nf;
   float* outp = a.out + (int64_t)dir * H * P;
-  float* gsave = a.gates ? a.gates + (int64_t)dir * 4 * H * P : nullptr;
-  float* csave = a.gates ? a.cstate + (int64_t)dir * H * P : nullptr;
+  f32x4* ssave = a.saved ? reinterpret_cast<f32x4*>(a.saved + (int64_t)dir * 5 * H * P) : nullptr;
   const int bufw = nks * 256;
   uint64_t* xch = a.xch + (int64_t)cluster * 2 * bufw;
   uint32_t* ctr = a.ctr + cluster * 16;
@@ -250,12 +252,17 @@
     }
     if (rvalid) {
 #pragma unroll
-      for (int r = 0; r < 8; ++r) {
-        const uint32_t o = o0 + (uint32_t)((r & 3) + 8 * (r >> 2)) * uP;
-        outp[o] = hv[r];
-        if (gsave) {
-          gsave[o] = gi[r]; gsave[o + HP] = gf[r]; gsave[o + 2 * HP] = gc[r]; gsave[o + 3 * HP] = go[r];
-          csave[o] = c[r];
+      for (int r = 0; r < 8; ++r) outp[o0 + (uint32_t)((r & 3) + 8 * (r >> 2)) * uP] = hv[r];
+      if (ssave) {
+#pragma unroll
+        for (int hb = 0; hb < 2; ++hb) {
+          const int r0 = 4 * hb;
+          f32x4* d = ssave + lstm_sv_idx(t, 4 * ub + 2 * hb + hh, H, Bn, row);
+          d[0] = f32x4{gi[r0], gi[r0 + 1], gi[r0 + 2], gi[r0 + 3]};
+          d[Bn] = f32x4{gf[r0], gf[r0 + 1], gf[r0 + 2], gf[r0 + 3]};
+          d[2 * Bn] = f32x4{gc[r0], gc[r0 + 1], gc[r0 + 2], gc[r0 + 3]};
+          d[3 * Bn] = f32x4{go[r0], go[r0 + 1], go[r0 + 2], go[r0 + 3]};
+          d[4 * Bn] = f32x4{c[r0], c[r0 + 1], c[r0 + 2], c[r0 + 3]};
         }
       }
     }
@@ -285,8 +292,7 @@
   uint64_t abase = (uint64_t)(a.packA + (int64_t)dir * a.pack_stride + 2 * nf + ub * 64);
   lstm_gptr_t Ahi = (lstm_gptr_t)abase;
   lstm_gptr_t Alo = Ahi + nb;
-  const float* __restrict__ gates = a.gates + (int64_t)dir * 4 * H * P;
-  const float* __restrict__ cst = a.cstate + (int64_t)dir * H * P;
+  const f32x4* __restrict__ sv = reinterpret_cast<const f32x4*>(a.saved + (int64_t)dir * 5 * H * P);
   float* __restrict__ dG = a.dG + (int64_t)dir * 4 * H * P;
   const float* __restrict__ goutp = a.gout + (int64_t)dir * H * P;
   const int bufw = nwv * nwv * 256;
@@ -305,17 +311,32 @@
   }
   float dcc[8], ct[8];
   float sg[4][8], cp[8], gy[8];
+  auto load_saved = [&](int tn, int tp) {
+#pragma unroll
+    for (int hb = 0; hb < 2; ++hb) {
+      const f32x4* q = sv + lstm_sv_idx(tn, 4 * ub + 2 * hb + hh, H, Bn, rowc);
+      const f32x4 v0 = q[0], v1 = q[Bn], v2 = q[2 * Bn], v3 = q[3 * Bn], vc = sv[lstm_sv_idx(tp, 4 * ub + 2 * hb + hh, H, Bn, rowc) + 4 * Bn];
+#pragma unroll
+      for (int e = 0; e < 4; ++e) {
+        sg[0][4 * hb + e] = v0[e]; sg[1][4 * hb + e] = v1[e]; sg[2][4 * hb + e] = v2[e]; sg[3][4 * hb + e] = v3[e];
+        cp[4 * hb + e] = vc[e];
+      }
+    }
+  };
   {
-    const uint32_t o0 = ubase + (uint32_t)((dir == 0 ? T - 1 : 0) * Bn);
-    const uint32_t op0 = ubase + (uint32_t)((T > 1 ? (dir == 0 ? T - 2 : 1) : (dir == 0 ? T - 1 : 0)) * Bn);
+    const int t0 = dir == 0 ? T - 1 : 0;
+    const uint32_t o0 = ubase + (uint32_t)(t0 * Bn);
+    load_saved(t0, T > 1 ? (dir == 0 ? T - 2 : 1) : t0);
+#pragma unroll
+    for (int hb = 0; hb < 2; ++hb) {
+      const f32x4 vc = sv[lstm_sv_idx(t0, 4 * ub + 2 * hb + hh, H, Bn, rowc) + 4 * Bn];
+#pragma unroll
+      for (int e = 0; e < 4; ++e) ct[4 * hb + e] = vc[e];
+    }
 #pragma unroll
     for (int r = 0; r < 8; ++r) {
-      const uint32_t du = (uint32_t)((r & 3) + 8 * (r >> 2)) * uP;
       dcc[r] = 0.f;
-      ct[r] = cst[o0 + du];
-      sg[0][r] = gates[o0 + du]; sg[1][r] = gates[o0 + du + HP]; sg[2][r] = gates[o0 + du + 2 * HP]; sg[3][r] = gates[o0 + du + 3 * HP];
-      cp[r] = cst[op0 + du];
-      gy[r] = goutp[o0 + du];
+      gy[r] = goutp[o0 + (uint32_t)((r & 3) + 8 * (r >> 2)) * uP];
     }
   }
   for (int s = T - 1; s >= 0; --s) {
@@ -441,14 +462,9 @@
     if (s > 0) {
       const int s1 = s - 1, s2 = s1 > 0 ? s1 - 1 : 0;
       const uint32_t on = ubase + (uint32_t)((dir == 0 ? s1 : T - 1 - s1) * Bn);
-      const uint32_t opn = ubase + (uint32_t)((dir == 0 ? s2 : T - 1 - s2) * Bn);
-#pragma unroll
-      for (int r = 0; r < 8; ++r) {
-        const uint32_t du = (uint32_t)((r & 3) + 8 * (r >> 2)) * uP;
-        sg[0][r] = gates[on + du]; sg[1][r] = gates[on + du + HP]; sg[2][r] = gates[on + du + 2 * HP]; sg[3][r] = gates[on + du + 3 * HP];
-        cp[r] = cst[opn + du];
-        gy[r] = goutp[on + du];
-      }
+      load_saved(dir == 0 ? s1 : T - 1 - s1, dir == 0 ? s2 : T - 1 - s2);
+#pragma unroll
+      for (int r = 0; r < 8; ++r) gy[r] = goutp[on + (uint32_t)((r & 3) + 8 * (r >> 2)) * uP];
     }
   }
 }
@@ -488,23 +504,58 @@
 }
 __device__ __forceinline__ void lstm_lds_barrier() { asm volatile("s_waitcnt lgkmcnt(0)\n\ts_barrier" ::: "memory"); }
 
-template <int NW>
+#define RFX_LSTM_TR_FLOATS (16 * 20)
+__device__ __forceinline__ void lstm_tr_put_units(float* m, int sq, int qb, const f32x4& v) {
+  *reinterpret_cast<f32x4*>(m + sq * 20 + 4 * qb) = v;
+}
+__device__ __forceinline__ f32x4 lstm_tr_get_units(const float* m, int sq, int qb) {
+  __builtin_amdgcn_wave_barrier();
+  return *reinterpret_cast<const f32x4*>(m + sq * 20 + 4 * qb);
+}
+__device__ __forceinline__ void lstm_tr_put_seqs(float* m, int tu, int tq, const f32x4& v) {
+#pragma unroll
+  for (int j = 0; j < 4; ++j) m[(4 * tq + j) * 20 + tu] = v[j];
+}
+__device__ __forceinline__ f32x4 lstm_tr_get_seqs(const float* m, int tu, int tq) {
+  __builtin_amdgcn_wave_barrier();
+  return f32x4{m[(4 * tq) * 20 + tu], m[(4 * tq + 1) * 20 + tu], m[(4 * tq + 2) * 20 + tu], m[(4 * tq + 3) * 20 + tu]};
+}
+template <bool VEC>
+__device__ __forceinline__ f32x4 lstm_row_load(const float* __restrict__ base, uint32_t o, int b0, int Bn) {
+  if (VEC) return rfx_ld4(base + (o + (uint32_t)(b0 < Bn ? b0 : 0)));
+  f32x4 v;
+#pragma unroll
+  for (int j = 0; j < 4; ++j) v[j] = base[o + (uint32_t)(b0 + j < Bn ? b0 + j : 0)];
+  return v;
+}
+template <bool VEC>
+__device__ __forceinline__ void lstm_row_store(float* base, uint32_t o, int b0, int Bn, const f32x4& v) {
+  if (VEC) {
+    if (b0 < Bn) rfx_st4(base + (o + (uint32_t)b0), v);
+    return;
+  }
+#pragma unroll
+  for (int j = 0; j < 4; ++j)
+    if (b0 + j < Bn) base[o + (uint32_t)(b0 + j)] = v[j];
+}
+
+template <int NW, bool VEC>
 __global__ __launch_bounds__(64 * NW) __attribute__((amdgpu_waves_per_eu(3, 3))) void lstm_fwd_local_kernel(const LstmArgs a, const uint4* __restrict__ lpack,
                                                                                                              int64_t lstride) {
   constexpr int H = 16 * NW, NK = H / 32;
   const int cluster = blockIdx.x, dir = cluster & 1, tile = cluster >> 1;
   const int tid = threadIdx.x, w = __builtin_amdgcn_readfirstlane(tid >> 6), lane = tid & 63, sq = lane & 15, qb = lane >> 4;
+  const int tu = lane & 15, tq = lane >> 4;
   const int Bn = a.Bn, T = a.T, P = a.P;
-  const int b = tile * 16 + sq;
+  const int b = tile * 16 + sq, b0 = tile * 16 + 4 * tq;
   const bool rvalid = b < Bn;
-  const int bc = rvalid ? b : 0;
   const float* __restrict__ xp = a.xp + (int64_t)dir * 4 * H * P;
   float* outp = a.out + (int64_t)dir * H * P;
-  float* gsave = a.gates ? a.gates + (int64_t)dir * 4 * H * P : nullptr;
-  float* csave = a.gates ? a.cstate + (int64_t)dir * H * P : nullptr;
+  f32x4* ssave = a.saved ? reinterpret_cast<f32x4*>(a.saved + (int64_t)dir * 5 * H * P) : nullptr;
   const uint32_t uP = (uint32_t)P, HP = (uint32_t)H * uP;
   const int u0 = 16 * w + 4 * qb;
-  const uint32_t ubase = (uint32_t)u0 * uP + (uint32_t)bc;
+  const uint32_t rbase = (uint32_t)(16 * w + tu) * uP;
+  float* tr = reinterpret_cast<float*>(lstm_smem + 2 * NK * 1024) + w * 5 * RFX_LSTM_TR_FLOATS;
   uint4 wf[4][NK];
   {
     const uint4* A = lpack + (int64_t)dir * lstride + (int64_t)w * 4 * NK * 64 + lane;
@@ -514,17 +565,14 @@
       for (int ks = 0; ks < NK; ++ks) wf[g][ks] = A[(g * NK + ks) * 64];
   }
   float c[4] = {0.f, 0.f, 0.f, 0.f};
-  float xpv[4][4];
-  {
-    const uint32_t o0 = ubase + (uint32_t)((dir == 0 ? 0 : T - 1) * Bn);
-#pragma unroll
-    for (int g = 0; g < 4; ++g)
-#pragma unroll
-      for (int r = 0; r < 4; ++r) xpv[g][r] = xp[o0 + (uint32_t)g * HP + (uint32_t)r * uP];
-  }
+  f32x4 xr[4];
+  auto load_xp = [&](int tn) {
+#pragma unroll
+    for (int g = 0; g < 4; ++g) xr[g] = lstm_row_load<VEC>(xp, (uint32_t)g * HP + rbase + (uint32_t)(tn * Bn), b0, Bn);
+  };
+  load_xp(dir == 0 ? 0 : T - 1);
   for (int s = 0; s < T; ++s) {
     const int t = dir == 0 ? s : T - 1 - s;
-    const uint32_t o0 = ubase + (uint32_t)(t * Bn);
     lstm_f32x4 acc[4];
 #pragma unroll
     for (int g = 0; g < 4; ++g) acc[g] = lstm_f32x4{0.f, 0.f, 0.f, 0.f};
@@ -538,6 +586,11 @@
           acc[g] = __builtin_amdgcn_mfma_f32_16x16x32_bf16(__builtin_bit_cast(bf16x8, wf[g][ks]), bh, acc[g], 0, 0, 0);
       }
     }
+    f32x4 xpv[4];
+#pragma unroll
+    for (int g = 0; g < 4; ++g) lstm_tr_put_seqs(tr + g * RFX_LSTM_TR_FLOATS, tu, tq, xr[g]);
+#pragma unroll
+    for (int g = 0; g < 4; ++g) xpv[g] = lstm_tr_get_units(tr + g * RFX_LSTM_TR_FLOATS, sq, qb);
     float hv[4], gi[4], gf[4], gc[4], go[4];
 #pragma unroll
     for (int r = 0; r < 4; ++r) {
@@ -549,68 +602,68 @@
     }
     if (s + 1 < T) {
       lstm_local_publish(lstm_smem + (s & 1) * (NK * 1024), u0, sq, hv[0], hv[1], hv[2], hv[3]);
-      const uint32_t on = ubase + (uint32_t)((dir == 0 ? s + 1 : T - 2 - s) * Bn);
-#pragma unroll
-      for (int g = 0; g < 4; ++g)
-#pragma unroll
-        for (int r = 0; r < 4; ++r) xpv[g][r] = xp[on + (uint32_t)g * HP + (uint32_t)r * uP];
+      load_xp(dir == 0 ? s + 1 : T - 2 - s);
       lstm_lds_barrier();
     }
-    if (rvalid) {
-#pragma unroll
-      for (int r = 0; r < 4; ++r) {
-        const uint32_t o = o0 + (uint32_t)r * uP;
-        outp[o] = hv[r];
-        if (gsave) {
-          gsave[o] = gi[r]; gsave[o + HP] = gf[r]; gsave[o + 2 * HP] = gc[r]; gsave[o + 3 * HP] = go[r];
-          csave[o] = c[r];
-        }
-      }
-    }
-  }
-}
-
-template <int NW>
+    float* to = tr + 4 * RFX_LSTM_TR_FLOATS;
+    lstm_tr_put_units(to, sq, qb, f32x4{hv[0], hv[1], hv[2], hv[3]});
+    lstm_row_store<VEC>(outp, rbase + (uint32_t)(t * Bn), b0, Bn, lstm_tr_get_seqs(to, tu, tq));
+    if (ssave && rvalid) {
+      const uint32_t o = lstm_sv_idx(t, u0 / 4, H, Bn, b), uB = (uint32_t)Bn;
+      ssave[o] = f32x4{gi[0], gi[1], gi[2], gi[3]};
+      ssave[o + uB] = f32x4{gf[0], gf[1], gf[2], gf[3]};
+      ssave[o + 2 * uB] = f32x4{gc[0], gc[1], gc[2], gc[3]};
+      ssave[o + 3 * uB] = f32x4{go[0], go[1], go[2], go[3]};
+      ssave[o + 4 * uB] = f32x4{c[0], c[1], c[2], c[3]};
+    }
+  }
+}
+
+template <int NW, bool VEC>
 __global__ __launch_bounds__(64 * NW) __attribute__((amdgpu_waves_per_eu(3, 3))) void lstm_bwd_local_kernel(const LstmArgs a, const uint4* __restrict__ lpack,
                                                                                                              int64_t lstride) {
   constexpr int H = 16 * NW, NK = H / 32, NK4 = 4 * NK;
   const int cluster = blockIdx.x, dir = cluster & 1, tile = cluster >> 1;
   const int tid = threadIdx.x, w = __builtin_amdgcn_readfirstlane(tid >> 6), lane = tid & 63, sq = lane & 15, qb = lane >> 4;
+  const int tu = lane & 15, tq = lane >> 4;
   const int Bn = a.Bn, T = a.T, P = a.P;
-  const int b = tile * 16 + sq;
-  const bool rvalid = b < Bn;
-  const int bc = rvalid ? b : 0;
-  const float* __restrict__ gates = a.gates + (int64_t)dir * 4 * H * P;
-  const float* __restrict__ cst = a.cstate + (int64_t)dir * H * P;
+  const int b = tile * 16 + sq, b0 = tile * 16 + 4 * tq;
+  const int bc = b < Bn ? b : 0;
+  const f32x4* __restrict__ sv = reinterpret_cast<const f32x4*>(a.saved + (int64_t)dir * 5 * H * P);
   float* __restrict__ dG = a.dG + (int64_t)dir * 4 * H * P;
   const float* __restrict__ goutp = a.gout + (int64_t)dir * H * P;
   const uint32_t uP = (uint32_t)P, HP = (uint32_t)H * uP;
   const int u0 = 16 * w + 4 * qb;
-  const uint32_t ubase = (uint32_t)u0 * uP + (uint32_t)bc;
+  const uint32_t rbase = (uint32_t)(16 * w + tu) * uP;
+  float* tr = reinterpret_cast<float*>(lstm_smem + 2 * NK4 * 1024) + w * 5 * RFX_LSTM_TR_FLOATS;
   uint4 wb[NK4];
   {
     const uint4* A = lpack + (int64_t)dir * lstride + (int64_t)NW * 4 * NK * 64 + (int64_t)w * NK4 * 64 + lane;
 #pragma unroll
     for (int ks = 0; ks < NK4; ++ks) wb[ks] = A[ks * 64];
   }
-  float dcc[4] = {0.f, 0.f, 0.f, 0.f}, ct[4], sg[4][4], cp[4], gy[4];
+  float dcc[4] = {0.f, 0.f, 0.f, 0.f}, ct[4], sg[4][4], cp[4];
+  f32x4 gr;
+  auto load_saved = [&](int tn, int tp) {
+    const uint32_t o = lstm_sv_idx(tn, u0 / 4, H, Bn, bc), uB = (uint32_t)Bn;
+    const f32x4 v0 = sv[o], v1 = sv[o + uB], v2 = sv[o + 2 * uB], v3 = sv[o + 3 * uB], vc = sv[lstm_sv_idx(tp, u0 / 4, H, Bn, bc) + 4 * uB];
+#pragma unroll
+    for (int r = 0; r < 4; ++r) { sg[0][r] = v0[r]; sg[1][r] = v1[r]; sg[2][r] = v2[r]; sg[3][r] = v3[r]; cp[r] = vc[r]; }
+  };
   {
-    const uint32_t o0 = ubase + (uint32_t)((dir == 0 ? T - 1 : 0) * Bn);
-    const uint32_t op0 = ubase + (uint32_t)((T > 1 ? (dir == 0 ? T - 2 : 1) : (dir == 0 ? T - 1 : 0)) * Bn);
-#pragma unroll
-    for (int r = 0; r < 4; ++r) {
-      const uint32_t du = (uint32_t)r * uP;
-      ct[r] = cst[o0 + du];
-      sg[0][r] = gates[o0 + du]; sg[1][r] = gates[o0 + du + HP]; sg[2][r] = gates[o0 + du + 2 * HP]; sg[3][r] = gates[o0 + du + 3 * HP];
-      cp[r] = cst[op0 + du];
-      gy[r] = goutp[o0 + du];
-    }
+    const int t0 = dir == 0 ? T - 1 : 0;
+    load_saved(t0, T > 1 ? (dir == 0 ? T - 2 : 1) : t0);
+    const f32x4 vc = sv[lstm_sv_idx(t0, u0 / 4, H, Bn, bc) + 4 * Bn];
+#pragma unroll
+    for (int r = 0; r < 4; ++r) ct[r] = vc[r];
+    gr = lstm_row_load<VEC>(goutp, rbase + (uint32_t)(t0 * Bn), b0, Bn);
   }
   lstm_f32x4 rec = lstm_f32x4{0.f, 0.f, 0.f, 0.f};
   for (int s = T - 1; s >= 0; --s) {
     const int step = T - 1 - s;
     const int t = dir == 0 ? s : T - 1 - s;
-    const uint32_t o0 = ubase + (uint32_t)(t * Bn);
+    lstm_tr_put_seqs(tr, tu, tq, gr);
+    const f32x4 gy = lstm_tr_get_units(tr, sq, qb);
 #pragma unroll
     for (int r = 0; r < 4; ++r) {
       const float dh = gy[r] + rec[r];
@@ -630,13 +683,11 @@
 #pragma unroll
       for (int g = 0; g < 4; ++g) lstm_local_publish(gb, g * H + u0, sq, sg[g][0], sg[g][1], sg[g][2], sg[g][3]);
     }
-    if (rvalid) {
-#pragma unroll
-      for (int r = 0; r < 4; ++r) {
-        const uint32_t o = o0 + (uint32_t)r * uP;
-        dG[o] = sg[0][r]; dG[o + HP] = sg[1][r]; dG[o + 2 * HP] = sg[2][r]; dG[o + 3 * HP] = sg[3][r];
-      }
-    }
+#pragma unroll
+    for (int g = 0; g < 4; ++g) lstm_tr_put_units(tr + (1 + g) * RFX_LSTM_TR_FLOATS, sq, qb, f32x4{sg[g][0], sg[g][1], sg[g][2], sg[g][3]});
+#pragma unroll
+    for (int g = 0; g < 4; ++g)
+      lstm_row_store<VEC>(dG, (uint32_t)g * HP + rbase + (uint32_t)(t * Bn), b0, Bn, lstm_tr_get_seqs(tr + (1 + g) * RFX_LSTM_TR_FLOATS, tu, tq));
     if (s > 0) {
       lstm_lds_barrier();
       lstm_f32x4 p[4];
@@ -648,15 +699,9 @@
         p[ks & 3] = __builtin_amdgcn_mfma_f32_16x16x32_bf16(__builtin_bit_cast(bf16x8, wb[ks]), bh, p[ks & 3], 0, 0, 0);
       }
       const int s1 = s - 1, s2 = s1 > 0 ? s1 - 1 : 0;
-      const uint32_t on = ubase + (uint32_t)((dir == 0 ? s1 : T - 1 - s1) * Bn);
-      const uint32_t opn = ubase + (uint32_t)((dir == 0 ? s2 : T - 1 - s2) * Bn);
-#pragma unroll
-      for (int r = 0; r < 4; ++r) {
-        const uint32_t du = (uint32_t)r * uP;
-        sg[0][r] = gates[on + du]; sg[1][r] = gates[on + du + HP]; sg[2][r] = gates[on + du + 2 * HP]; sg[3][r] = gates[on + du + 3 * HP];
-        cp[r] = cst[opn + du];
-        gy[r] = goutp[on + du];
-      }
+      const int tn = dir == 0 ? s1 : T - 1 - s1;
+      load_saved(tn, dir == 0 ? s2 : T - 1 - s2);
+      gr = lstm_row_load<VEC>(goutp, rbase + (uint32_t)(tn * Bn), b0, Bn);
       rec = (p[0] + p[1]) + (p[2] + p[3]);
     }
   }
@@ -673,8 +718,8 @@
   if (m[0] < 0) {
     const char* e = getenv("RFX_LSTM_LOCAL");
     const char* eb = getenv("RFX_LSTM_LOCAL_BWD");
-    m[0] = e ? atoi(e) : 64;
-    m[1] = m[0] > 0 ? (eb ? atoi(eb) : 16) : 0;
+    m[0] = e ? atoi(e) : 0;
+    m[1] = m[0] > 0 ? (eb ? atoi(eb) : 0) : 0;
   }
   return m[bwd];
 }
@@ -691,15 +736,20 @@
   const int ntiles = (a.Bn + 15) / 16;
   const uint4* lpack = a.packA + lstm_cluster_uint4_per_dir(H);
   const int64_t lstride = a.pack_stride;
-  const size_t smem = (size_t)2 * (bwd ? 4 : 1) * (H / 32) * 1024;
-  static bool attr[2] = {false, false};
-  if (!attr[bwd]) {
-    const void* k = bwd ? reinterpret_cast<const void*>(&lstm_bwd_local_kernel<NW>) : reinterpret_cast<const void*>(&lstm_fwd_local_kernel<NW>);
+  const size_t smem = (size_t)2 * (bwd ? 4 : 1) * (H / 32) * 1024 + (size_t)NW * 5 * RFX_LSTM_TR_FLOATS * 4;
+  auto al16 = [](const void* p) { return (reinterpret_cast<uintptr_t>(p) & 15) == 0; };
+  const bool vec = (a.Bn & 3) == 0 && (bwd ? al16(a.gout) && al16(a.dG) : al16(a.xp) && al16(a.out));
+  const void* k = bwd ? (vec ? reinterpret_cast<const void*>(&lstm_bwd_local_kernel<NW, true>) : reinterpret_cast<const void*>(&lstm_bwd_local_kernel<NW, false>))
+                      : (vec ? reinterpret_cast<const void*>(&lstm_fwd_local_kernel<NW, true>) : reinterpret_cast<const void*>(&lstm_fwd_local_kernel<NW, false>));
+  static bool attr[4] = {false, false, false, false};
+  if (!attr[2 * bwd + vec]) {
     if (hipFuncSetAttribute(k, hipFuncAttributeMaxDynamicSharedMemorySize, (int)smem) != hipSuccess) return -3;
-    attr[bwd] = true;
-  }
-  if (bwd) hipLaunchKernelGGL((lstm_bwd_local_kernel<NW>), dim3(2 * ntiles), dim3(64 * NW), smem, s, a, lpack, lstride);
-  else hipLaunchKernelGGL((lstm_fwd_local_kernel<NW>), dim3(2 * ntiles), dim3(64 * NW), smem, s, a, lpack, lstride);
+    attr[2 * bwd + vec] = true;
+  }
+  if (bwd && vec) hipLaunchKernelGGL((lstm_bwd_local_kernel<NW, true>), dim3(2 * ntiles), dim3(64 * NW), smem, s, a, lpack, lstride);
+  else if (bwd) hipLaunchKernelGGL((lstm_bwd_local_kernel<NW, false>), dim3(2 * ntiles), dim3(64 * NW), smem, s, a, lpack, lstride);
+  else if (vec) hipLaunchKernelGGL((lstm_fwd_local_kernel<NW, true>), dim3(2 * ntiles), dim3(64 * NW), smem, s, a, lpack, lstride);
+  else hipLaunchKernelGGL((lstm_fwd_local_kernel<NW, false>), dim3(2 * ntiles), dim3(64 * NW), smem, s, a, lpack, lstride);
   RFX_CHECK_LAUNCH();
   return 0;
 }
@@ -833,12 +883,12 @@
 }
 
 extern "C" int rfx_lstm_fwd(const float* xp, const void* pack, int32_t T, int32_t Bn, int32_t H, float* out,
-                            float* gates, float* cstate, void* ws, int32_t prec, void* stream) {
+                            float* saved, void* ws, int32_t prec, void* stream) {
   if (!xp || !pack || !out || !ws || T <= 0 || Bn <= 0 || lstm_bad_h(H)) return -1;
-  if ((gates == nullptr) != (cstate == nullptr)) return -1;
   if ((int64_t)4 * H * T * Bn >= ((int64_t)1 << 31)) return -1;
+  if (saved && (reinterpret_cast<uintptr_t>(saved) & 15)) return -1;
   LstmArgs a{};
-  a.xp = xp; a.packA = reinterpret_cast<const uint4*>(pack); a.out = out; a.gates = gates; a.cstate = cstate;
+  a.xp = xp; a.packA = reinterpret_cast<const uint4*>(pack); a.out = out; a.saved = saved;
   a.pack_stride = lstm_pack_uint4_per_dir(H); a.T = T; a.Bn = Bn; a.H = H; a.P = T * Bn;
   const int wf = H / 16;
   if (lstm_local_ok(H, prec, Bn, false)) return lstm_local_launch<12>(false, a, (hipStream_t)stream);
@@ -855,13 +905,13 @@
   return H % 64 == 0 ? lstm_launch(lstm_fwd_kernel<4, 0, true>, a, wf, ws, stream) : lstm_launch(lstm_fwd_kernel<2, 0, true>, a, wf, ws, stream);
 }
 
-extern "C" int rfx_lstm_bwd(const float* gout, const void* pack, const float* gates, const float* cstate, int32_t T,
+extern "C" int rfx_lstm_bwd(const float* gout, const void* pack, const float* saved, int32_t T,
                             int32_t Bn, int32_t H, float* dG, void* ws, int32_t prec, void* stream) {
-  if (!gout || !pack || !gates || !cstate || !dG || !ws || T <= 0 || Bn <= 0 || lstm_bad_h(H)) return -1;
+  if (!gout || !pack || !saved || !dG || !ws || T <= 0 || Bn <= 0 || lstm_bad_h(H)) return -1;
   if ((int64_t)4 * H * T * Bn >= ((int64_t)1 << 31)) return -1;
+  if (reinterpret_cast<uintptr_t>(saved) & 15) return -1;
   LstmArgs a{};
-  a.gout = gout; a.packA = reinterpret_cast<const uint4*>(pack); a.gates = const_cast<float*>(gates);
-  a.cstate = const_cast<float*>(cstate); a.dG = dG;
+  a.gout = gout; a.packA = reinterpret_cast<const uint4*>(pack); a.saved = const_cast<float*>(saved); a.dG = dG;
   a.pack_stride = lstm_pack_uint4_per_dir(H); a.T = T; a.Bn = Bn; a.H = H; a.P = T * Bn;
   const int wb = H / 16;
   if (lstm_local_ok(H, prec, Bn, true)) return lstm_local_launch<12>(true, a, (hipStream_t)stream);
diff --git a/remfx_amd/lstm.py b/remfx_amd/lstm.py
--- a/remfx_amd/lstm.py
+++ b/remfx_amd/lstm.py
@@ -78,26 +78,25 @@
         need = any(ctx.needs_input_grad)
         pack = _pack_whh(w_hh, w_hh_r, Bn, need)
         out = torch.empty((1, 2 * H, P), device=x.device, dtype=torch.float32)
-        gates = torch.empty((2, 4 * H, P), device=x.device, dtype=torch.float32) if need else None
-        cst = torch.empty((2, H, P), device=x.device, dtype=torch.float32) if need else None
-        check(_lib.lib().rfx_lstm_fwd(_ptr(xp), _ptr(pack), T, Bn, H, _ptr(out), _ptr(gates), _ptr(cst),
+        saved = torch.empty((2, 5 * H, P), device=x.device, dtype=torch.float32) if need else None
+        check(_lib.lib().rfx_lstm_fwd(_ptr(xp), _ptr(pack), T, Bn, H, _ptr(out), _ptr(saved),
                                       _ptr(_workspace(x.device, H)), ops.GEMM_PREC, _stream()),
               "rfx_lstm_fwd")
         ctx.prec = ops.GEMM_PREC
         if need:
-            ctx.save_for_backward(x, wcat, pack, gates, cst, out)
+            ctx.save_for_backward(x, wcat, pack, saved, out)
             ctx.dims = (T, Bn, H, Cin)
             ctx.params = (w_ih, w_hh, b_ih, b_hh, w_ih_r, w_hh_r, b_ih_r, b_hh_r)
         return out
 
     @staticmethod
     def backward(ctx, g):
-        x, wcat, pack, gates, cst, out = ctx.saved_tensors
+        x, wcat, pack, saved, out = ctx.saved_tensors
         T, Bn, H, Cin = ctx.dims
         P = T * Bn
         g = g.contiguous()
         dG = torch.empty((1, 8 * H, 1, P), device=g.device, dtype=torch.float32)
-        check(_lib.lib().rfx_lstm_bwd(_ptr(g), _ptr(pack), _ptr(gates), _ptr(cst), T, Bn, H, _ptr(dG),
+        check(_lib.lib().rfx_lstm_bwd(_ptr(g), _ptr(pack), _ptr(saved), T, Bn, H, _ptr(dG),
                                       _ptr(_workspace(g.device, H)), ctx.prec, _stream()),
               "rfx_lstm_bwd")
         x4 = x.unsqueeze(2)
```

Result: no change. 3698 audio-seconds/sec (median of 6 runs) (+0.6%).
